# jaak-s/libfastsparse

Measured on AMD Instinct MI355X. Metric: fp64 CSR SpMV effective GB/s (% HBM3E peak), higher is better.
Workload: dtype f64

## Files before the change

libfastsparse_amd/csrc/fs_copies.hip:

```cpp
#include <algorithm>
#include <vector>

#include "fs_format_util.h"
#include "fs_plan.h"

namespace fs {

static_assert(sizeof(WorkItem) == sizeof(int4) && sizeof(RowLen) == sizeof(int2), "fs_plan.h's plain structs are the device's int4 / int2");

__global__ void piece_count_kernel(int nrow, int split, const int *__restrict__ row_ptr, int *__restrict__ cnt)
{
  const int r = blockIdx.x * blockDim.x + threadIdx.x;
  if (r > nrow) return;
  if (r == nrow) { cnt[r] = 0; return; }
  const int len = row_ptr[r + 1] - row_ptr[r];
  cnt[r] = len <= split ? 1 : (len + split - 1) / split;
}

__global__ void vrow_fill_kernel(int nrow, int split, const int *__restrict__ row_ptr, const int *__restrict__ vfirst,
                                 int *__restrict__ vrow_ptr)
{
  const int r = blockIdx.x * blockDim.x + threadIdx.x;
  if (r > nrow) return;
  if (r == nrow) { vrow_ptr[vfirst[nrow]] = row_ptr[nrow]; return; }
  const int a = row_ptr[r], v0 = vfirst[r], k = vfirst[r + 1] - v0;
  for (int i = 0; i < k; ++i) vrow_ptr[v0 + i] = a + i * split;
}

__device__ __forceinline__ int last_le(const int *__restrict__ a, int n, int64_t key)
{
  int lo = 0, hi = n;
  while (lo < hi) {
    const int mid = lo + ((hi - lo + 1) >> 1);
    if ((int64_t)a[mid] <= key) lo = mid; else hi = mid - 1;
  }
  return lo;
}

__global__ void tile_key_kernel(int nvrow, int64_t nnz, int P, int W, int J, const int *__restrict__ vrow_ptr,
                                const int *__restrict__ panel_row, const int *__restrict__ cols,
                                int *__restrict__ vrows, unsigned *__restrict__ keys)
{
  const int64_t i = (int64_t)blockIdx.x * blockDim.x + threadIdx.x;
  if (i >= nnz) return;
  const int v = last_le(vrow_ptr, nvrow, i);
  vrows[i] = v;
  const int p = last_le(panel_row, P, v);
  keys[i] = (unsigned)p * (unsigned)J + (unsigned)(cols[i] / W);
}

__global__ void tile_pack_kernel(int64_t nnz, int W, int J, int lcol_bits, const unsigned *__restrict__ skeys,
                                 const unsigned *__restrict__ perm, const int *__restrict__ vrows,
                                 const int *__restrict__ panel_row, const int *__restrict__ cols,
                                 const double *__restrict__ vals, unsigned *__restrict__ pk, double *__restrict__ vals_out)
{
  const int64_t i = (int64_t)blockIdx.x * blockDim.x + threadIdx.x;
  if (i >= nnz) return;
  const unsigned src = perm[i];
  const unsigned key = skeys[i];
  const unsigned p = key / (unsigned)J, j = key % (unsigned)J;
  const unsigned lrow = (unsigned)(vrows[src] - panel_row[p]), lcol = (unsigned)(cols[src] - (int)j * W);
  pk[i] = (lrow << lcol_bits) | lcol;
  if (vals) vals_out[i] = vals[src];
}

__global__ void max_row_len_kernel(int nrow, const int *__restrict__ row_ptr, int *__restrict__ out)
{
  const int r = blockIdx.x * blockDim.x + threadIdx.x;
  int len = r < nrow ? row_ptr[r + 1] - row_ptr[r] : 0;
  for (int m = 32; m > 0; m >>= 1) { const int o = __shfl_xor(len, m); len = o > len ? o : len; }
  if ((threadIdx.x & 63) == 0 && len > __hip_atomic_load(out, __ATOMIC_RELAXED, __HIP_MEMORY_SCOPE_AGENT)) atomicMax(out, len);
}

static int make_virtual_rows(const DeviceCsr &A, int split, hipStream_t s, Scratch<int> &vrow_ptr, int *nvrow_out,
                             int **vfirst_out, double **yv_out, int kw = 1)
{
  Scratch<int> cnt;
  Scratch<char> tmp;
  int nvrow = 0;
  FS_HIP(cnt.alloc((size_t)A.nrow + 1));
  FS_HIP(traced_malloc(vfirst_out, sizeof(int) * ((size_t)A.nrow + 1)));
  int *vfirst = *vfirst_out;
  hipLaunchKernelGGL(piece_count_kernel, dim3(grid_for((int64_t)A.nrow + 1)), dim3(256), 0, s, A.nrow, split, A.row_ptr,
                     cnt.p);
  FS_HIP(hipGetLastError());
  if (int rc = device_exclusive_scan(tmp, cnt.p, vfirst, (size_t)A.nrow + 1, s)) return rc;
  if (int rc = read_back(&nvrow, (const int *)vfirst + A.nrow, s)) return rc;
  FS_HIP(vrow_ptr.alloc((size_t)nvrow + 1));
  hipLaunchKernelGGL(vrow_fill_kernel, dim3(grid_for((int64_t)A.nrow + 1)), dim3(256), 0, s, A.nrow, split, A.row_ptr,
                     vfirst, vrow_ptr.p);
  FS_HIP(hipGetLastError());
  FS_HIP(traced_malloc(yv_out, sizeof(double) * (size_t)nvrow * (size_t)kw));
  *nvrow_out = nvrow;
  return FS_OK;
}

static int max_row_len(const DeviceCsr &A, hipStream_t s, int *out)
{
  if (A.max_row_len >= 0) { *out = A.max_row_len; return FS_OK; }
  Scratch<int> mx;
  FS_HIP(mx.alloc(1));
  FS_HIP(hipMemsetAsync(mx, 0, sizeof(int), s));
  hipLaunchKernelGGL(max_row_len_kernel, dim3(grid_for(A.nrow)), dim3(256), 0, s, A.nrow, A.row_ptr, mx.p);
  FS_HIP(hipGetLastError());
  if (int rc = read_back(out, (const int *)mx.p, s)) return rc;
  A.max_row_len = *out;
  return FS_OK;
}

struct VirtualRows {
  Scratch<int> own;
  const int *vrow_ptr = nullptr;
  int nvrow = 0;
  int split = 0;
  bool cut() const { return split > 0; }
  int fetch(std::vector<int> &vp, hipStream_t s) const
  {
    vp.resize((size_t)nvrow + 1);
    FS_HIP(hipMemcpyAsync(vp.data(), vrow_ptr, sizeof(int) * vp.size(), hipMemcpyDeviceToHost, s));
    FS_HIP(hipStreamSynchronize(s));
    return FS_OK;
  }
};

static int virtual_rows(const DeviceCsr &A, hipStream_t s, bool may_cut, int kw, VirtualRows &V, int **vfirst, double **yv)
{
  int max_len = 0;
  if (int rc = max_row_len(A, s, &max_len)) return rc;
  const int split = options().tile_split > 0 ? options().tile_split : 256;
  V.vrow_ptr = A.row_ptr;
  V.nvrow = A.nrow;
  if (may_cut && max_len > split) {
    V.split = split;
    if (int rc = make_virtual_rows(A, split, s, V.own, &V.nvrow, vfirst, yv, kw)) return rc;
    V.vrow_ptr = V.own.p;
  }
  return FS_OK;
}

static int sorted_runs(Scratch<char> &tmp, unsigned *keys, unsigned *skeys, unsigned *idx_in, unsigned *idx_out, size_t n, int64_t nruns,
                       int *run_ptr, hipStream_t s, const unsigned **sorted_keys, const unsigned **perm)
{
  if (int rc = device_iota((int64_t)n, idx_in, s)) return rc;
  if (int rc = device_sort_pairs(tmp, keys, skeys, idx_in, idx_out, n, sort_bits((uint64_t)nruns, 32), s, sorted_keys, perm)) return rc;
  return device_run_ptr(nruns, (int64_t)n, *sorted_keys, run_ptr, s);
}

__device__ __forceinline__ int rot_ffs(unsigned m, int rot)
{
  const unsigned rr = rot ? ((m >> rot) | (m << (32 - rot))) : m;
  return (__ffs((int)rr) - 1 + rot) & 31;
}

__device__ __forceinline__ void wave_lds_fence()
{
  __builtin_amdgcn_fence(__ATOMIC_SEQ_CST, "workgroup");
  __builtin_amdgcn_wave_barrier();
}

constexpr int kReorderThreads = 256;
constexpr int kReorderSegs = kReorderThreads / 32;
constexpr int kReorderPer = kTiledItem / kReorderThreads;

constexpr int kRepairMaxClass = 256;
constexpr int kRepairMaxGroup = 8;
constexpr int kRepairMaxLeft = 128;
constexpr int kRepairMaxBig = 96;

template <bool ARRANGE>
__global__ __launch_bounds__(kReorderThreads) void ldsx_reorder_kernel(const int4 *__restrict__ items, int lcol_bits,
                                                                      unsigned *__restrict__ pk, double *__restrict__ vals,
                                                                      int *__restrict__ bad, unsigned long long *__restrict__ clk)
{
  long long tick = clk ? clock64() : 0;
  auto lap = [&](int phase) {
    if (clk && threadIdx.x == 0) { const long long now = clock64(); atomicAdd(&clk[phase], (unsigned long long)(now - tick)); tick = now; }
  };
  __shared__ unsigned w[kTiledItem];
  __shared__ unsigned short lst[kTiledItem];
  __shared__ unsigned short seq[kTiledItem];
  __shared__ unsigned short segcnt[kReorderSegs][32 * 32];
  __shared__ unsigned short left[32 * 32];
  __shared__ unsigned short size[32 * 32];
  __shared__ unsigned short off[32 * 32];
  __shared__ int owner[32];
  static_assert(kReorderSegs * 32 * 32 >= 3 * kTiledItem + kTiledItem / 2, "the repair arrays are carved out of segcnt");
  unsigned short *const cplace = &segcnt[0][0];
  unsigned short *const crow = &segcnt[0][0] + kTiledItem;
  unsigned short *const lead = &segcnt[0][0] + 2 * kTiledItem;
  unsigned char *const flag = reinterpret_cast<unsigned char *>(&segcnt[0][0] + 3 * kTiledItem);
  __shared__ unsigned short unres[kRepairMaxLeft];
  __shared__ unsigned short pmem[kRepairMaxBig];
  __shared__ int nunres, ndup, wcount[32];
  const int4 d = items[blockIdx.x];
  const int n = d.y, t = threadIdx.x;
  for (int i = t; i < n; i += kReorderThreads) w[i] = pk[(int64_t)d.x + i];
  for (int i = t; i < kReorderSegs * 32 * 32; i += kReorderThreads) (&segcnt[0][0])[i] = 0;
  __syncthreads();
  {
    const int sg = t >> 5, c = t & 31;
    const int per = (n + kReorderSegs - 1) / kReorderSegs;
    const int i0 = sg * per, i1 = (i0 + per < n) ? i0 + per : n;
    for (int i = i0; i < i1; ++i)
      if ((int)((w[i] >> lcol_bits) & 31u) == c) {
        const int k = c * 32 + (ARRANGE ? (int)(w[i] & 31u) : 0);
        seq[i] = segcnt[sg][k]++;
      }
  }
  __syncthreads();
  lap(0);
  for (int k = t; k < 32 * 32; k += kReorderThreads) {
    int a = 0;
    for (int sg = 0; sg < kReorderSegs; ++sg) { const int m = segcnt[sg][k]; segcnt[sg][k] = (unsigned short)a; a += m; }
    size[k] = (unsigned short)a;
    left[k] = (unsigned short)a;
  }
  __syncthreads();
  unsigned avail = 0;
  int mine = 0;
  if (t < 64) {
    if (t < 32)
      for (int b = 0; b < 32; ++b) mine += size[t * 32 + b];
    int base = mine;
    for (int m = 1; m < 32; m <<= 1) {
      const int o = __shfl_up(base, m);
      if (t >= m) base += o;
    }
    base -= mine;
    if (t < 32) {
      int a = base;
      for (int b = 0; b < 32; ++b) {
        off[t * 32 + b] = (unsigned short)a;
        a += size[t * 32 + b];
        if (size[t * 32 + b]) avail |= 1u << b;
      }
    }
  }
  __syncthreads();
  {
    const int per = (n + kReorderSegs - 1) / kReorderSegs;
    for (int i = t; i < n; i += kReorderThreads) {
      const int k = (int)((w[i] >> lcol_bits) & 31u) * 32 + (ARRANGE ? (int)(w[i] & 31u) : 0);
      lst[off[k] + segcnt[i / per][k] + seq[i]] = (unsigned short)i;
    }
  }
  __syncthreads();
  lap(1);
  if (t < 64) {
    int remaining = t < 32 ? mine : 0, placed = 0;
    for (int r = 0;; ++r) {
      const unsigned nonempty = (unsigned)__ballot(remaining > 0);
      if (!nonempty) break;
      unsigned used = 0;
      int bank = -1;
      bool pending = remaining > 0;
      for (int iter = 0;; ++iter) {
        int prop = -1;
        if (pending) {
          const unsigned free_banks = avail & ~used;
          const int rot = (t + r + 7 * iter) & 31;
          if (!ARRANGE || free_banks == 0u) { bank = rot_ffs(avail, rot); pending = false; }
          else prop = rot_ffs(free_banks, rot);
        }
        if (!__ballot(prop >= 0)) break;
        if (t < 32) owner[t] = 255;
        wave_lds_fence();
        if (prop >= 0) atomicMin(&owner[prop], t);
        wave_lds_fence();
        if (prop >= 0 && owner[prop] == t) { bank = prop; pending = false; }
        used |= (unsigned)__ballot(t < 32 && owner[t & 31] != 255);
        wave_lds_fence();
      }
      if (bank >= 0) {
        const int k = t * 32 + bank;
        const int before = left[k];
        left[k] = (unsigned short)(before - 1);
        if (before == 1) avail &= ~(1u << bank);
        const int place = placed + __popc(nonempty & ((1u << t) - 1u));
        seq[place] = lst[off[k] + (size[k] - before)];
        cplace[off[t * 32] + (mine - remaining)] = (unsigned short)place;
        --remaining;
      }
      placed += __popc(nonempty);
    }
  }
  __syncthreads();
  lap(2);
  const int half = (n + 1) >> 1;
  {
    for (int g = t; g < n; g += kReorderThreads) crow[g] = (unsigned short)(w[seq[cplace[g]]] >> lcol_bits);
    __syncthreads();
    bool too_large = false;
    const int wv = __builtin_amdgcn_readfirstlane(t >> 6), lane = t & 63;
    auto rdlane = [](int v, int l) { return __builtin_amdgcn_readlane(v, __builtin_amdgcn_readfirstlane(l)); };
    for (int q8 = 0; q8 < 8; ++q8) {
      const int c = wv * 8 + q8;
      const int base = __builtin_amdgcn_readfirstlane((int)off[c * 32]);
      const int msize = __builtin_amdgcn_readfirstlane((c < 31 ? (int)off[(c + 1) * 32] : n) - base);
      const int m = msize < kRepairMaxClass ? msize : kRepairMaxClass;
      int row[4];
#pragma unroll
      for (int e = 0; e < 4; ++e) {
        const int idx = 64 * e + lane;
        row[e] = idx < m ? (int)crow[base + idx] : -1 - idx;
      }
#pragma unroll
      for (int e = 0; e < 4; ++e) {
        if (64 * e < m) {
          int first = -1;
#pragma unroll
          for (int e2 = 0; e2 < 4; ++e2) {
            if (e2 <= e) {
              const int lim = e2 < e ? 64 : lane;
              const int cnt = m - 64 * e2 < 64 ? m - 64 * e2 : 64;
              for (int l = 0; l < cnt; ++l) {
                const int rl = rdlane(row[e2], l);
                if (first < 0 && rl == row[e] && l < lim) first = 64 * e2 + l;
              }
            }
          }
          const int idx = 64 * e + lane;
          if (idx < m) {
            lead[base + idx] = (unsigned short)(base + (first < 0 ? idx : first));
            flag[base + idx] = 0;
          }
        }
      }
      for (int idx = kRepairMaxClass + lane; idx < msize; idx += 64) {
        lead[base + idx] = (unsigned short)(base + idx);
        flag[base + idx] = 0;
        too_large = true;
      }
    }
    __syncthreads();
    if (t == 0) { nunres = 0; ndup = 0; }
    __syncthreads();
    {
      int mydup = 0;
      for (int g = t; g < n; g += kReorderThreads)
        if (lead[g] != g) { flag[lead[g]] = 1; ++mydup; }
      if (mydup) atomicAdd(&ndup, mydup);
    }
    __syncthreads();
    lap(3);
    const bool hopeless = 4 * ndup > n && n > 128;
    bool failed = too_large || hopeless;
    auto wave_of = [&](int g) { const int sp = cplace[g]; return (sp < half ? sp : sp - half) >> 6; };
    auto trade = [&](int j, int k, int g) {
      const unsigned short ej = seq[cplace[j]], ek = seq[cplace[k]];
      seq[cplace[j]] = ek; seq[cplace[k]] = ej;
      const unsigned short rj = crow[j]; crow[j] = crow[k]; crow[k] = rj;
      lead[k] = (unsigned short)g; flag[k] = 2;
      lead[j] = (unsigned short)j; flag[j] = 0;
    };
    if (!hopeless) {
      for (int q8 = 0; q8 < 8; ++q8) {
        const int c = wv * 8 + q8;
        const int base = __builtin_amdgcn_readfirstlane((int)off[c * 32]);
        const int msize = __builtin_amdgcn_readfirstlane((c < 31 ? (int)off[(c + 1) * 32] : n) - base);
        const int m = msize < kRepairMaxClass ? msize : kRepairMaxClass;
        if (m <= 0) continue;
        int wof[4];
#pragma unroll
        for (int e = 0; e < 4; ++e) wof[e] = 64 * e + lane < m ? wave_of(base + 64 * e + lane) : 31;
        int myfree = 0;
        {
          bool fr[4];
#pragma unroll
          for (int e = 0; e < 4; ++e) {
            const int g = base + 64 * e + lane;
            fr[e] = 64 * e + lane < m && lead[g] == g && !(flag[g] & 3);
          }
          for (int v = 0; v < 16; ++v) {
            int cnt = 0;
#pragma unroll
            for (int e = 0; e < 4; ++e) cnt += __popcll(__ballot(fr[e] && wof[e] == v));
            if (lane == v) myfree = cnt;
          }
        }
        int cursor = -1;
        for (;;) {
          int G = -1;
#pragma unroll
          for (int e = 0; e < 4; ++e) {
            const int idx = 64 * e + lane, g = base + idx;
            const bool d = idx < m && idx > cursor && lead[g] == g && (flag[g] & 1) && !(flag[g] & 2);
            const unsigned long long mk = __ballot(d);
            if (G < 0 && mk) G = 64 * e + __ffsll((long long)mk) - 1;
          }
          if (G < 0) break;
          cursor = G;
          const int gG = base + G;
          bool mem[4];
          int gs = 0;
#pragma unroll
          for (int e = 0; e < 4; ++e) {
            mem[e] = 64 * e + lane < m && lead[base + 64 * e + lane] == gG;
            gs += __popcll(__ballot(mem[e]));
          }
          int best = -1;
          if (gs <= kRepairMaxGroup) {
            int have = 0;
#pragma unroll
            for (int e = 0; e < 4; ++e) {
              unsigned long long bits = __ballot(mem[e]);
              while (bits) {
                const int l = __ffsll((long long)bits) - 1;
                bits &= bits - 1;
                if (lane == rdlane(wof[e], l)) ++have;
              }
            }
            int key = (lane < 16 && have + myfree >= gs) ? ((have << 8) | (15 - lane)) : -1;
            for (int o = 32; o > 0; o >>= 1) { const int other = __shfl_xor(key, o); key = other > key ? other : key; }
            if (key >= 0) best = 15 - (key & 255);
          }
          if (best < 0) {
            if (lane == 0) {
              const int slot = atomicAdd(&nunres, 1);
              if (slot < kRepairMaxLeft) unres[slot] = (unsigned short)gG; else failed = true;
            }
            continue;
          }
#pragma unroll
          for (int e = 0; e < 4; ++e) {
            unsigned long long bits = __ballot(mem[e]);
            while (bits) {
              const int l = __ffsll((long long)bits) - 1;
              bits &= bits - 1;
              const int j = base + 64 * e + l;
              const int wj = rdlane(wof[e], l);
              if (wj == best) {
                if (lane == 0) flag[j] |= 2;
                wave_lds_fence();
                continue;
              }
              int k = -1;
#pragma unroll
              for (int e2 = 0; e2 < 4; ++e2) {
                const int g2 = base + 64 * e2 + lane;
                const bool f = 64 * e2 + lane < m && wof[e2] == best && lead[g2] == g2 && !(flag[g2] & 3);
                const unsigned long long fm = __ballot(f);
                if (k < 0 && fm) k = base + 64 * e2 + __ffsll((long long)fm) - 1;
              }
              if (k < 0) { failed = true; break; }
              if (lane == 0) trade(j, k, gG);
              wave_lds_fence();
              if (lane == best) --myfree;
              if (lane == wj) ++myfree;
            }
          }
          wave_lds_fence();
        }
      }
    }
    __syncthreads();
    {
      const int cnt = nunres < kRepairMaxLeft ? nunres : kRepairMaxLeft;
      int mine_u = 0, rank = 0;
      if (t < cnt) {
        mine_u = unres[t];
        for (int j = 0; j < cnt; ++j) rank += unres[j] < mine_u;
      }
      __syncthreads();
      if (t < cnt) unres[rank] = (unsigned short)mine_u;
    }
    __syncthreads();
    lap(4);
    {
      const int left = hopeless ? 0 : (nunres < kRepairMaxLeft ? nunres : kRepairMaxLeft);
      if (!hopeless && nunres > kRepairMaxLeft) failed = true;
      for (int u = 0; u < left; ++u) {
        const int g = unres[u];
        if (t < 32) wcount[t] = 0;
        __syncthreads();
        for (int j = t; j < n; j += kReorderThreads) {
          const int v = wave_of(j);
          if (lead[j] == g) atomicAdd(&wcount[v], 1);
          else if (lead[j] == j && !(flag[j] & 3)) atomicAdd(&wcount[16 + v], 1);
        }
        __syncthreads();
        if (t == 0 && !failed) {
          const int c = crow[g] & 31, base = off[c * 32];
          int m = (c < 31 ? (int)off[(c + 1) * 32] : n) - base;
          if (m > kRepairMaxClass) m = kRepairMaxClass;
          int gs = 0;
          for (int j = g; j < base + m; ++j)
            if (lead[j] == g) { if (gs < kRepairMaxBig) pmem[gs] = (unsigned short)j; ++gs; }
          int best = -1;
          for (int v = 0; v < 16; ++v)
            if (wcount[v] + wcount[16 + v] >= gs && (best < 0 || wcount[v] > wcount[best])) best = v;
          if (gs > kRepairMaxBig || best < 0) failed = true;
          else {
            int next = 0;
            for (int q = 0; q < gs; ++q) {
              const int j = pmem[q];
              if (wave_of(j) == best) { flag[j] |= 2; continue; }
              while (next < n && !(wave_of(next) == best && lead[next] == next && !(flag[next] & 3))) ++next;
              if (next >= n) { failed = true; break; }
              trade(j, next, g);
            }
          }
        }
        __syncthreads();
      }
    }
    if (failed) atomicAdd(bad, 1);
  }
  __syncthreads();
  lap(5);
  double v[kReorderPer];
#pragma unroll
  for (int j = 0; j < kReorderPer; ++j) {
    const int q = t + j * kReorderThreads;
    v[j] = (vals && q < n) ? vals[(int64_t)d.x + seq[q]] : 0.0;
  }
  __syncthreads();
#pragma unroll
  for (int j = 0; j < kReorderPer; ++j) {
    const int q = t + j * kReorderThreads;
    if (q < n) {
      const int pos = q < half ? 2 * q : 2 * (q - half) + 1;
      pk[(int64_t)d.x + pos] = w[seq[q]];
      if (vals) vals[(int64_t)d.x + pos] = v[j];
    }
  }
  lap(6);
}

constexpr int kPanelBandWords = 8192;
__global__ __launch_bounds__(256) void panel_bands_kernel(int stride, int W, int words, const int *__restrict__ panel_row,
                                                          const int *__restrict__ row_ptr, const int *__restrict__ cols,
                                                          int *__restrict__ out)
{
  __shared__ unsigned bits[kPanelBandWords];
  __shared__ int total;
  const int p = blockIdx.x * stride, t = threadIdx.x;
  for (int i = t; i < words; i += 256) bits[i] = 0u;
  if (t == 0) total = 0;
  __syncthreads();
  const int64_t e0 = row_ptr[panel_row[p]], e1 = row_ptr[panel_row[p + 1]];
  for (int64_t e = e0 + t; e < e1; e += 256) {
    const int b = cols[e] / W;
    atomicOr(&bits[b >> 5], 1u << (b & 31));
  }
  __syncthreads();
  int c = 0;
  for (int i = t; i < words; i += 256) c += __popc(bits[i]);
  atomicAdd(&total, c);
  __syncthreads();
  if (t == 0) { out[2 * blockIdx.x] = total; out[2 * blockIdx.x + 1] = (int)(e1 - e0); }
}

static int ldsx_sample_is_thin(const DeviceCsr &A, const int *vrow_ptr, const std::vector<int> &panel_row, int W, int J, hipStream_t s,
                               bool *thin)
{
  *thin = true;
  constexpr int kSample = 64;
  const int P = (int)panel_row.size() - 1, words = (J + 31) / 32;
  if (words > kPanelBandWords || P < 1) return FS_OK;
  const int ns = P < kSample ? P : kSample, stride = P / ns;
  Scratch<int> prow, cnt;
  FS_HIP(prow.alloc(panel_row.size()));
  FS_HIP(cnt.alloc(2 * (size_t)ns));
  FS_HIP(hipMemcpyAsync(prow.p, panel_row.data(), sizeof(int) * panel_row.size(), hipMemcpyHostToDevice, s));
  hipLaunchKernelGGL(panel_bands_kernel, dim3(ns), dim3(256), 0, s, stride, W, words, prow.p, vrow_ptr, A.cols, cnt.p);
  FS_HIP(hipGetLastError());
  std::vector<int> hc(2 * (size_t)ns);
  FS_HIP(hipMemcpyAsync(hc.data(), cnt.p, sizeof(int) * hc.size(), hipMemcpyDeviceToHost, s));
  FS_HIP(hipStreamSynchronize(s));
  *thin = ldsx_sample_thin(hc);
  return FS_OK;
}

static int reorder_ldsx_items(TiledCsr *T, hipStream_t s)
{
  static const bool arrange = [] { const char *v = getenv("FS_LDSX_ARRANGE"); return !(v && *v == '0'); }();
  static const bool profile = [] { const char *v = getenv("FS_LDSX_REORDER_PROFILE"); return v && *v == '1'; }();
  Scratch<int> bad;
  Scratch<unsigned long long> clk;
  FS_HIP(bad.alloc(1));
  FS_HIP(hipMemsetAsync(bad, 0, sizeof(int), s));
  if (profile) { FS_HIP(clk.alloc(8)); FS_HIP(hipMemsetAsync(clk, 0, 8 * sizeof(unsigned long long), s)); }
  if (arrange)
    hipLaunchKernelGGL(ldsx_reorder_kernel<true>, dim3(T->nitems), dim3(kReorderThreads), 0, s, T->items, T->lcol_bits, T->pk, T->vals, bad.p, profile ? clk.p : nullptr);
  else
    hipLaunchKernelGGL(ldsx_reorder_kernel<false>, dim3(T->nitems), dim3(kReorderThreads), 0, s, T->items, T->lcol_bits, T->pk, T->vals, bad.p, profile ? clk.p : nullptr);
  FS_HIP(hipGetLastError());
  if (profile) {
    unsigned long long h[8] = {};
    FS_HIP(hipMemcpyAsync(h, clk, sizeof h, hipMemcpyDeviceToHost, s));
    FS_HIP(hipStreamSynchronize(s));
    fprintf(stderr, "[fastsparse] ldsx_reorder_kernel, %d items, mean clocks per item: load+count %.0f, lists %.0f, rounds %.0f, repair rows+leaders %.0f, "
            "per class %.0f, leftovers %.0f, copy out %.0f\n", T->nitems, (double)h[0] / T->nitems, (double)h[1] / T->nitems, (double)h[2] / T->nitems,
            (double)h[3] / T->nitems, (double)h[4] / T->nitems, (double)h[5] / T->nitems, (double)h[6] / T->nitems);
  }
  int hbad = 0;
  if (int rc = read_back(&hbad, bad.p, s)) return rc;
  T->orderable = hbad == 0;
  if (trace_build() && hbad) fprintf(stderr, "[fastsparse] LDS-staged copy: %d of %d work items hold a row that does not fit one wave -- no fixed-order sums on this copy\n", hbad, T->nitems);
  return FS_OK;
}

static int upload_ldsx_chunks(TiledCsr *T, int nrow, const std::vector<int> &chunk_panel, const std::vector<int> &chunk_item,
                              const std::vector<int> &chunk_ord)
{
  const int P = T->P;
  T->nchunks = (int)chunk_panel.size();
  FS_HIP(traced_malloc(&T->chunk_panel, sizeof(int) * (chunk_panel.size() ? chunk_panel.size() : 1)));
  FS_HIP(traced_malloc(&T->chunk_item, sizeof(int) * (chunk_item.size() ? chunk_item.size() : 2)));
  FS_HIP(traced_malloc(&T->chunk_ord, sizeof(int) * (chunk_ord.size() ? chunk_ord.size() : 1)));
  {
    int *base = nullptr;
    FS_HIP(traced_malloc(&base, sizeof(int) * ((size_t)(P > 0 ? P : 1) + 1)));
    FS_HIP(hipMemset(base, 0, sizeof(int)));
    T->ticket = base + 1;
  }
  if (!chunk_panel.empty()) {
    FS_HIP(hipMemcpy(T->chunk_panel, chunk_panel.data(), sizeof(int) * chunk_panel.size(), hipMemcpyHostToDevice));
    FS_HIP(hipMemcpy(T->chunk_item, chunk_item.data(), sizeof(int) * chunk_item.size(), hipMemcpyHostToDevice));
    FS_HIP(hipMemcpy(T->chunk_ord, chunk_ord.data(), sizeof(int) * chunk_ord.size(), hipMemcpyHostToDevice));
  }
  if (T->shared && !T->yv) FS_HIP(traced_malloc(&T->yv, sizeof(double) * (size_t)nrow));
  return FS_OK;
}

static int build_tiled_impl(DeviceCsr &A, hipStream_t s, TiledCsr *&slot, bool ldsx)
{
  const Options &o = options();
  const int mode = ldsx ? o.ldsx : o.tiling;
  if (mode == 0 || A.nrow == 0 || A.nnz == 0) return FS_OK;
  const int ncu = cu_count();
  const int slots = (ncu > 8 ? ncu : 256) / 8 * 8;
  const int rows_max = ldsx ? kLdsxRows : kTiledRowsMax;

  const int64_t x_bytes = (int64_t)A.ncol * 8;
  if (mode == 1 && tiled_too_small(x_bytes, A.nnz)) return FS_OK;

  TiledCsr *T = new TiledCsr();
  slot = T;
  T->ldsx = ldsx;
  T->slots = slots; T->lcol_bits = kTiledColBits;
  VirtualRows V;
  if (int rc = virtual_rows(A, s, !ldsx, 1, V, &T->vfirst, &T->yv)) return rc;
  T->split = V.split;
  T->nvrow = V.nvrow;

  const int R = plan_tiled_rows(V.nvrow, slots, rows_max, ldsx, o.tile_rows);
  std::vector<int> vp;
  if (V.cut())
    if (int rc = V.fetch(vp, s)) return rc;
  const std::vector<int> panel_row = plan_tiled_panels(V.nvrow, R, V.cut(), vp, A.nnz, V.split);
  const int P = (int)panel_row.size() - 1;
  int W = 0, J = 0;
  plan_band_width(A.ncol, A.nnz, P, ldsx, o.tile_cols, &W, &J);
  const int64_t ntiles = (int64_t)P * J;
  if (mode == 1 && ldsx && ldsx_tiles_thin(A.nnz, ntiles)) {
    bool thin = true;
    if (int rc = ldsx_sample_is_thin(A, V.vrow_ptr, panel_row, W, J, s, &thin)) return rc;
    if (thin) return FS_OK;
  }
  if (mode == 1 && !ldsx && tiled_hopeless(A.nnz, ntiles, P, slots, x_bytes)) return FS_OK;
  if (ntiles >= (1ll << 31)) return FS_OK;
  T->R = R; T->W = W; T->P = P; T->J = J;
  T->entries_per_tile = (float)((double)A.nnz / (double)ntiles);
  FS_HIP(traced_malloc(&T->panel_row, sizeof(int) * panel_row.size()));
  FS_HIP(hipMemcpyAsync(T->panel_row, panel_row.data(), sizeof(int) * panel_row.size(), hipMemcpyHostToDevice, s));

  const size_t n = (size_t)A.nnz;
  Scratch<int> vrows, tile_ptr;
  Scratch<unsigned> keys, skeys, idx_in, idx_out;
  Scratch<char> tmp;
  FS_HIP(vrows.alloc(n));
  FS_HIP(keys.alloc(n));
  FS_HIP(skeys.alloc(n));
  FS_HIP(idx_in.alloc(n));
  FS_HIP(idx_out.alloc(n));
  FS_HIP(tile_ptr.alloc((size_t)ntiles + 1));
  FS_HIP(traced_malloc(&T->pk, sizeof(unsigned) * (n + 8)));
  if (A.vals) FS_HIP(traced_malloc(&T->vals, sizeof(double) * (n + 8)));
  hipLaunchKernelGGL(tile_key_kernel, dim3(grid_for(A.nnz)), dim3(256), 0, s, V.nvrow, A.nnz, P, W, J, V.vrow_ptr, T->panel_row,
                     A.cols, vrows.p, keys.p);
  const unsigned *sorted_keys = nullptr, *perm = nullptr;
  if (int rc = sorted_runs(tmp, keys.p, skeys.p, idx_in.p, idx_out.p, n, ntiles, tile_ptr.p, s, &sorted_keys, &perm)) return rc;
  hipLaunchKernelGGL(tile_pack_kernel, dim3(grid_for(A.nnz)), dim3(256), 0, s, A.nnz, W, J, T->lcol_bits, sorted_keys, perm,
                     vrows.p, T->panel_row, A.cols, A.vals, T->pk, T->vals);
  FS_HIP(hipGetLastError());
  std::vector<int> tp((size_t)ntiles + 1);
  FS_HIP(hipMemcpyAsync(tp.data(), tile_ptr.p, sizeof(int) * tp.size(), hipMemcpyDeviceToHost, s));
  FS_HIP(hipStreamSynchronize(s));
  std::vector<WorkItem> items;
  std::vector<int> item_ptr;
  cut_work_items(tp, P, J, items, item_ptr);
  T->nitems = (int)items.size();
  FS_HIP(traced_malloc(&T->items, sizeof(int4) * (items.size() ? items.size() : 1)));
  FS_HIP(traced_malloc(&T->item_ptr, sizeof(int) * item_ptr.size()));
  if (!items.empty()) FS_HIP(hipMemcpy(T->items, items.data(), sizeof(int4) * items.size(), hipMemcpyHostToDevice));
  FS_HIP(hipMemcpy(T->item_ptr, item_ptr.data(), sizeof(int) * item_ptr.size(), hipMemcpyHostToDevice));
  if (ldsx && T->nitems > 0)
    if (int rc = reorder_ldsx_items(T, s)) return rc;
  if (ldsx) {
    static const bool plain = [] { const char *v = getenv("FS_LDSX_ORDER"); return v && *v == '1'; }();
    std::vector<int> chunk_panel, chunk_item, chunk_ord;
    T->shared = plan_ldsx_chunks(item_ptr, (int64_t)items.size(), P, slots, plain, chunk_panel, chunk_item, chunk_ord);
    if (int rc = upload_ldsx_chunks(T, A.nrow, chunk_panel, chunk_item, chunk_ord)) return rc;
  }
  T->built = true;
  return FS_OK;
}

int build_tiled(DeviceCsr &A, hipStream_t s) { return optional_copy(build_tiled_impl(A, s, A.tiled, false), A.tiled, free_tiled_slot); }

int build_tiledx(DeviceCsr &A, hipStream_t s) { return optional_copy(build_tiled_impl(A, s, A.tiledx, true), A.tiledx, free_tiled_slot); }

__global__ void bin_key_kernel(int nvrow, int64_t nnz, int P, int bcols, const int *__restrict__ vrow_ptr,
                               const int *__restrict__ panel_row, const int *__restrict__ cols,
                               int *__restrict__ vrows, unsigned *__restrict__ keys)
{
  const int64_t i = (int64_t)blockIdx.x * blockDim.x + threadIdx.x;
  if (i >= nnz) return;
  const int v = last_le(vrow_ptr, nvrow, i);
  vrows[i] = v;
  keys[i] = (unsigned)(cols[i] / bcols) * (unsigned)P + (unsigned)last_le(panel_row, P, v);
}

__global__ void bin_groups_kernel(int B, int P, int ge, const int *__restrict__ run_ptr, unsigned *__restrict__ g1,
                                  unsigned *__restrict__ g2, const unsigned *__restrict__ xs = nullptr)
{
  const int64_t k = (int64_t)blockIdx.x * blockDim.x + threadIdx.x;
  const int64_t nruns = (int64_t)B * P;
  if (k > nruns) return;
  if (k == nruns) { g1[k] = 0; g2[k] = 0; return; }
  const int b = (int)(k / P), p = (int)(k % P);
  const unsigned dum = xs ? xs[run_ptr[k + 1]] - xs[run_ptr[k]] : 0u;
  const unsigned g = ((unsigned)(run_ptr[k + 1] - run_ptr[k]) + dum + (unsigned)ge - 1u) / (unsigned)ge;
  g1[k] = g;
  g2[(int64_t)p * B + b] = g;
}

__global__ void bin_scatter_kernel(int64_t nnz, int B, int P, int bcols, int ge, const unsigned *__restrict__ skeys,
                                   const unsigned *__restrict__ perm, const int *__restrict__ vrows,
                                   const int *__restrict__ panel_row, const int *__restrict__ cols,
                                   const double *__restrict__ vals, const int *__restrict__ run_ptr,
                                   const unsigned *__restrict__ start1, const unsigned *__restrict__ start2,
                                   uint16_t *__restrict__ lcol, double *__restrict__ vals1, uint16_t *__restrict__ lrow)
{
  const int64_t i = (int64_t)blockIdx.x * blockDim.x + threadIdx.x;
  if (i >= nnz) return;
  const unsigned key = skeys[i], src = perm[i];
  const int b = (int)(key / (unsigned)P), p = (int)(key % (unsigned)P);
  const int64_t rank = i - run_ptr[key];
  const int64_t pos1 = (int64_t)start1[key] * ge + rank;
  const int64_t pos2 = (int64_t)start2[(int64_t)p * B + b] * ge + rank;
  lcol[pos1] = (uint16_t)(cols[src] - b * bcols);
  if (vals) vals1[pos1] = vals[src];
  lrow[pos2] = (uint16_t)(vrows[src] - panel_row[p]);
}

__global__ void bin_gap_kernel(int64_t nnz, int P, const unsigned *__restrict__ skeys, const unsigned *__restrict__ perm,
                               const int *__restrict__ vrows, const int *__restrict__ run_ptr, unsigned *__restrict__ extra)
{
  const int64_t i = (int64_t)blockIdx.x * blockDim.x + threadIdx.x;
  if (i > nnz) return;
  if (i == nnz) { extra[i] = 0; return; }
  const unsigned key = skeys[i];
  unsigned e = 0;
  if (i > run_ptr[key]) {
    const int gap = vrows[perm[i]] - vrows[perm[i - 1]];
    if (gap > 255) e = (unsigned)(gap - 1) / 255u;
  }
  extra[i] = e;
}

__global__ void bin_scatter8_kernel(int64_t nnz, int B, int P, int bcols, int ge, const unsigned *__restrict__ skeys,
                                    const unsigned *__restrict__ perm, const int *__restrict__ vrows,
                                    const int *__restrict__ panel_row, const int *__restrict__ cols,
                                    const double *__restrict__ vals, const int *__restrict__ run_ptr,
                                    const unsigned *__restrict__ xs, const unsigned *__restrict__ start1,
                                    const unsigned *__restrict__ start2, uint16_t *__restrict__ lcol, double *__restrict__ vals1,
                                    uint8_t *__restrict__ lrow8, uint16_t *__restrict__ gbase)
{
  const int64_t i = (int64_t)blockIdx.x * blockDim.x + threadIdx.x;
  if (i >= nnz) return;
  const unsigned key = skeys[i], src = perm[i];
  const int b = (int)(key / (unsigned)P), p = (int)(key % (unsigned)P);
  const int64_t first = run_ptr[key];
  const unsigned dum = xs[i + 1] - xs[i];
  const int64_t slot = (i - first) + (int64_t)(xs[i] - xs[first]) + dum;
  const int64_t base1 = (int64_t)start1[key] * ge, base2 = (int64_t)start2[(int64_t)p * B + b] * ge;
  const int row = vrows[src] - panel_row[p];
  const int prev = i > first ? vrows[perm[i - 1]] - panel_row[p] : row;
  for (unsigned m = 0; m < dum; ++m) {
    const int64_t sl = slot - dum + m;
    lrow8[base2 + sl] = 255;
    if ((sl & (ge - 1)) == 0) gbase[(base2 + sl) / ge] = (uint16_t)(prev + 255 * (int)m);
  }
  const int before = prev + 255 * (int)dum;
  lcol[base1 + slot] = (uint16_t)(cols[src] - b * bcols);
  if (vals) vals1[base1 + slot] = vals[src];
  lrow8[base2 + slot] = (uint8_t)(row - before);
  if ((slot & (ge - 1)) == 0) gbase[(base2 + slot) / ge] = (uint16_t)before;
}

__global__ void bin_gdst_kernel(int B, int P, const unsigned *__restrict__ start1, const unsigned *__restrict__ start2,
                                unsigned *__restrict__ gdst)
{
  const int64_t k = (int64_t)blockIdx.x * blockDim.x + threadIdx.x;
  if (k >= (int64_t)B * P) return;
  const int b = (int)(k / P), p = (int)(k % P);
  const unsigned a = start1[k], n = start1[k + 1] - a, d = start2[(int64_t)p * B + b];
  for (unsigned j = 0; j < n; ++j) gdst[a + j] = d + j;
}

__global__ void bin_ptr_kernel(int B, int P, const unsigned *__restrict__ start1, const unsigned *__restrict__ start2,
                               unsigned *__restrict__ band_ptr, unsigned *__restrict__ bin_ptr)
{
  const int64_t k = (int64_t)blockIdx.x * blockDim.x + threadIdx.x;
  if (k <= B) band_ptr[k] = start1[k * P];
  if (k <= P) bin_ptr[k] = start2[k * B];
}

__global__ void long_candidates_kernel(int nrow, int minlen, const int *__restrict__ row_ptr, int *__restrict__ count, int cap,
                                       int2 *__restrict__ out)
{
  const int r = blockIdx.x * blockDim.x + threadIdx.x;
  if (r >= nrow) return;
  const int len = row_ptr[r + 1] - row_ptr[r];
  if (len < minlen) return;
  const int k = atomicAdd(count, 1);
  if (k < cap) out[k] = make_int2(r, len);
}

__global__ void long_mark_kernel(int nlong, const int *__restrict__ rows, int *__restrict__ row_to_long)
{
  const int i = blockIdx.x * blockDim.x + threadIdx.x;
  if (i < nlong) row_to_long[rows[i]] = i;
}

__global__ void main_len_kernel(int nrow, const int *__restrict__ row_ptr, const int *__restrict__ row_to_long, int *__restrict__ len)
{
  const int r = blockIdx.x * blockDim.x + threadIdx.x;
  if (r > nrow) return;
  len[r] = (r == nrow || row_to_long[r] >= 0) ? 0 : row_ptr[r + 1] - row_ptr[r];
}

__global__ void split_entries_kernel(int nrow, int64_t nnz, int nlong, int bcols, const int *__restrict__ row_ptr, const int *__restrict__ cols,
                                     const double *__restrict__ vals, const int *__restrict__ row_to_long,
                                     const int *__restrict__ main_rp, const int64_t *__restrict__ long_ptr,
                                     int *__restrict__ main_cols, double *__restrict__ main_vals, unsigned *__restrict__ lkey,
                                     unsigned *__restrict__ lsrc)
{
  const int64_t i = (int64_t)blockIdx.x * blockDim.x + threadIdx.x;
  if (i >= nnz) return;
  const int r = last_le(row_ptr, nrow, i);
  const int64_t k = i - row_ptr[r];
  const int l = row_to_long[r];
  if (l < 0) {
    const int64_t d = (int64_t)main_rp[r] + k;
    main_cols[d] = cols[i];
    if (vals) main_vals[d] = vals[i];
  } else {
    const int64_t d = long_ptr[l] + k;
    lkey[d] = (unsigned)(cols[i] / bcols) * (unsigned)nlong + (unsigned)l;
    lsrc[d] = (unsigned)i;
  }
}

__global__ void long_seg_start_kernel(int B, int nlong, int64_t n, const int *__restrict__ own_first, const unsigned *__restrict__ skeys,
                                      int64_t *__restrict__ start)
{
  const int64_t sg = (int64_t)blockIdx.x * blockDim.x + threadIdx.x;
  if (sg > (int64_t)B * kLongOwners) return;
  const int b = (int)(sg / kLongOwners), w = (int)(sg % kLongOwners);
  const uint64_t key = (uint64_t)b * (uint64_t)nlong + (uint64_t)(b < B ? own_first[w] : 0);
  int64_t lo = 0, hi = n;
  while (lo < hi) {
    const int64_t mid = lo + ((hi - lo) >> 1);
    if ((uint64_t)skeys[mid] < key) lo = mid + 1; else hi = mid;
  }
  start[sg] = lo;
}

__global__ void long_scatter_kernel(int64_t n, int nlong, int bcols, const unsigned *__restrict__ skeys, const unsigned *__restrict__ ssrc,
                                    const unsigned char *__restrict__ owner_of, const int64_t *__restrict__ shift,
                                    const int *__restrict__ cols, const double *__restrict__ vals, uint16_t *__restrict__ lcol,
                                    uint16_t *__restrict__ lrow, double *__restrict__ lvals)
{
  const int64_t k = (int64_t)blockIdx.x * blockDim.x + threadIdx.x;
  if (k >= n) return;
  const unsigned key = skeys[k], src = ssrc[k];
  const unsigned b = key / (unsigned)nlong, l = key - b * (unsigned)nlong;
  const int64_t d = k + shift[(int64_t)b * kLongOwners + owner_of[l]];
  lcol[d] = (uint16_t)(cols[src] - (int)b * bcols);
  lrow[d] = (uint16_t)l;
  if (lvals) lvals[d] = vals[src];
}

__global__ void long_pad_kernel(int64_t nseg, int bcols, const int64_t *__restrict__ start, const int64_t *__restrict__ shift,
                                uint16_t *__restrict__ lcol, uint16_t *__restrict__ lrow, double *__restrict__ lvals)
{
  const int64_t sg = (int64_t)blockIdx.x * blockDim.x + threadIdx.x;
  if (sg >= nseg) return;
  const int64_t cnt = start[sg + 1] - start[sg];
  if (cnt & 1) {
    const int64_t d = start[sg] + shift[sg] + cnt;
    lcol[d] = (uint16_t)bcols;
    lrow[d] = lrow[d - 1];
    if (lvals) lvals[d] = 0.0;
  }
}

static int split_long_rows(const DeviceCsr &A, hipStream_t s, LongRows **out, Scratch<int> &main_rp, Scratch<int> &main_cols,
                           Scratch<double> &main_vals, int64_t *main_nnz)
{
  *out = nullptr;
  const Options &o = options();
  if (o.long_rows == 0 || o.binning == 0 || A.nrow == 0 || A.nnz < (4 << 20)) return FS_OK;
  const bool narrow = o.long_geometry != 1;
  const int bcols = narrow ? kLongBandB : kLongBandA, cap_rows = narrow ? kLongRowsB : kLongRowsA;
  const int B = (A.ncol + bcols - 1) / bcols;
  const int minlen = o.long_min_len > 0 ? o.long_min_len : 512;
  constexpr int kCap = 1 << 18;
  Scratch<int> cnt;
  Scratch<int2> cand;
  FS_HIP(cnt.alloc(1));
  FS_HIP(cand.alloc(kCap));
  FS_HIP(hipMemsetAsync(cnt, 0, sizeof(int), s));
  hipLaunchKernelGGL(long_candidates_kernel, dim3(grid_for(A.nrow)), dim3(256), 0, s, A.nrow, minlen, A.row_ptr, cnt.p, kCap, cand.p);
  FS_HIP(hipGetLastError());
  int ncand = 0;
  if (int rc = read_back(&ncand, cnt.p, s)) return rc;
  if (ncand == 0 || ncand > kCap) return FS_OK;
  std::vector<RowLen> h((size_t)ncand);
  FS_HIP(hipMemcpy(h.data(), cand, sizeof(int2) * (size_t)ncand, hipMemcpyDeviceToHost));
  std::vector<int> rows, own_first;
  std::vector<unsigned char> owner_of;
  std::vector<int64_t> lptr;
  deal_long_rows(std::move(h), cap_rows, rows, own_first, owner_of, lptr);
  const int nlong = (int)rows.size();
  const int64_t nl = lptr[(size_t)nlong];
  if (o.long_rows == 1 && !long_rows_pay(nl, A.nnz, A.ncol)) return FS_OK;
  if ((uint64_t)B * (uint64_t)nlong >= (1ull << 32)) return FS_OK;

  LongRows *L = new LongRows();
  struct Guard { LongRows *&p; bool keep = false; ~Guard() { if (!keep) free_long_rows(p); } } guard{L};
  L->nlong = nlong; L->B = B; L->bcols = bcols;
  FS_HIP(traced_malloc(&L->row, sizeof(int) * (size_t)nlong));
  FS_HIP(hipMemcpyAsync(L->row, rows.data(), sizeof(int) * (size_t)nlong, hipMemcpyHostToDevice, s));
  FS_HIP(traced_malloc(&L->ylong, sizeof(double) * (size_t)nlong));

  Scratch<int> row_to_long, mlen;
  Scratch<int64_t> long_ptr, start, shift;
  Scratch<unsigned> lkey, lsrc, skey, ssrc;
  Scratch<char> tmp;
  FS_HIP(row_to_long.alloc((size_t)A.nrow));
  FS_HIP(mlen.alloc((size_t)A.nrow + 1));
  FS_HIP(main_rp.alloc((size_t)A.nrow + 1));
  FS_HIP(long_ptr.alloc((size_t)nlong + 1));
  FS_HIP(hipMemsetAsync(row_to_long, 0xff, sizeof(int) * (size_t)A.nrow, s));
  FS_HIP(hipMemcpyAsync(long_ptr, lptr.data(), sizeof(int64_t) * lptr.size(), hipMemcpyHostToDevice, s));
  hipLaunchKernelGGL(long_mark_kernel, dim3(grid_for(nlong)), dim3(256), 0, s, nlong, L->row, row_to_long.p);
  hipLaunchKernelGGL(main_len_kernel, dim3(grid_for((int64_t)A.nrow + 1)), dim3(256), 0, s, A.nrow, A.row_ptr, row_to_long.p, mlen.p);
  FS_HIP(hipGetLastError());
  if (int rc = device_exclusive_scan(tmp, mlen.p, main_rp.p, (size_t)A.nrow + 1, s)) return rc;
  const int64_t nm = A.nnz - nl;
  *main_nnz = nm;
  FS_HIP(main_cols.alloc((size_t)(nm > 0 ? nm : 1)));
  if (A.vals) FS_HIP(main_vals.alloc((size_t)(nm > 0 ? nm : 1)));
  FS_HIP(lkey.alloc((size_t)nl));
  FS_HIP(lsrc.alloc((size_t)nl));
  FS_HIP(skey.alloc((size_t)nl));
  FS_HIP(ssrc.alloc((size_t)nl));
  hipLaunchKernelGGL(split_entries_kernel, dim3(grid_for(A.nnz)), dim3(256), 0, s, A.nrow, A.nnz, nlong, bcols, A.row_ptr, A.cols, A.vals,
                     row_to_long.p, main_rp.p, long_ptr.p, main_cols.p, A.vals ? main_vals.p : nullptr, lkey.p, lsrc.p);
  FS_HIP(hipGetLastError());
  Scratch<char> tmp2;
  const unsigned *sorted_keys = nullptr, *sorted_src = nullptr;
  if (int rc = device_sort_pairs(tmp2, lkey.p, skey.p, lsrc.p, ssrc.p, (size_t)nl, sort_bits((uint64_t)B * (uint64_t)nlong, 32), s,
                                 &sorted_keys, &sorted_src)) return rc;
  const int64_t nseg = (int64_t)B * kLongOwners;
  Scratch<int> d_own_first;
  Scratch<unsigned char> d_owner_of;
  FS_HIP(start.alloc((size_t)nseg + 1));
  FS_HIP(shift.alloc((size_t)nseg + 1));
  FS_HIP(d_own_first.alloc((size_t)kLongOwners + 1));
  FS_HIP(d_owner_of.alloc((size_t)nlong));
  FS_HIP(hipMemcpyAsync(d_own_first, own_first.data(), sizeof(int) * own_first.size(), hipMemcpyHostToDevice, s));
  FS_HIP(hipMemcpyAsync(d_owner_of, owner_of.data(), owner_of.size(), hipMemcpyHostToDevice, s));
  hipLaunchKernelGGL(long_seg_start_kernel, dim3(grid_for(nseg + 1)), dim3(256), 0, s, B, nlong, nl, d_own_first.p, sorted_keys, start.p);
  FS_HIP(hipGetLastError());
  std::vector<int64_t> hs((size_t)nseg + 1), hp, hsh;
  std::vector<unsigned> hseg;
  FS_HIP(hipMemcpyAsync(hs.data(), start, sizeof(int64_t) * hs.size(), hipMemcpyDeviceToHost, s));
  FS_HIP(hipStreamSynchronize(s));
  if (!pad_long_segments(hs, B, hp, hseg, hsh)) return FS_OK;
  L->n = hp[(size_t)B];
  FS_HIP(traced_malloc(&L->band_ptr, sizeof(int64_t) * ((size_t)B + 1)));
  FS_HIP(traced_malloc(&L->seg_ptr, sizeof(unsigned) * hseg.size()));
  FS_HIP(hipMemcpyAsync(L->band_ptr, hp.data(), sizeof(int64_t) * hp.size(), hipMemcpyHostToDevice, s));
  FS_HIP(hipMemcpyAsync(L->seg_ptr, hseg.data(), sizeof(unsigned) * hseg.size(), hipMemcpyHostToDevice, s));
  FS_HIP(hipMemcpyAsync(shift, hsh.data(), sizeof(int64_t) * hsh.size(), hipMemcpyHostToDevice, s));
  FS_HIP(traced_malloc(&L->lcol, sizeof(uint16_t) * (size_t)(L->n + 2)));
  FS_HIP(traced_malloc(&L->lrow, sizeof(uint16_t) * (size_t)(L->n + 2)));
  if (A.vals) FS_HIP(traced_malloc(&L->vals, sizeof(double) * (size_t)(L->n + 2)));
  hipLaunchKernelGGL(long_scatter_kernel, dim3(grid_for(nl)), dim3(256), 0, s, nl, nlong, bcols, sorted_keys, sorted_src, d_owner_of.p,
                     shift.p, A.cols, A.vals, L->lcol, L->lrow, L->vals);
  hipLaunchKernelGGL(long_pad_kernel, dim3(grid_for(nseg)), dim3(256), 0, s, nseg, bcols, start.p, shift.p, L->lcol, L->lrow, L->vals);
  FS_HIP(hipGetLastError());
  const int ncu = cu_count();
  const int64_t by_size = (L->n + kBinShareMin - 1) / kBinShareMin;
  L->nwg = (int)(by_size < ncu ? by_size : ncu);
  FS_HIP(traced_malloc(&L->ypart, sizeof(double) * (size_t)(L->nwg > 0 ? L->nwg : 1) * (size_t)nlong));
  FS_HIP(hipStreamSynchronize(s));
  guard.keep = true;
  *out = L;
  return FS_OK;
}

static int build_binned_impl(DeviceCsr &A, hipStream_t s, BinnedCsr *&slot, int kw)
{
  const Options &o = options();
  static const int big_env = [] { const char *v = getenv("FS_BIN_BIG"); return v && *v ? atoi(v) : -1; }();
  const TwoPassGeometry g = plan_two_pass_geometry(A.nrow, A.ncol, A.nnz, kw, o.bin_rows, big_env);
  const int bcols = g.bcols, ge = g.ge;
  if (o.binning == 0 || A.nrow == 0 || A.nnz == 0) return FS_OK;
  if (o.binning == 1 && A.nnz < (4 << 20)) return FS_OK;
  const int ncu = cu_count();
  const int slots = ncu > 0 ? ncu : 256;

  BinnedCsr *N = new BinnedCsr();
  slot = N;
  N->kw = kw;
  N->bcols = bcols;
  VirtualRows V;
  if (int rc = virtual_rows(A, s, true, kw, V, &N->vfirst, &N->yv)) return rc;
  N->split = V.split;
  N->nvrow = V.nvrow;
  const int nvrow = V.nvrow;

  std::vector<int> vp;
  if (int rc = V.fetch(vp, s)) return rc;
  static const double fill = [] { const char *v = getenv("FS_BIN_FILL"); return v && *v ? atof(v) / 100.0 : 0.8; }();
  static const int min_panels = [] { const char *v = getenv("FS_BIN_MIN_PANELS"); return v && *v ? atoi(v) : 1; }();
  const std::vector<int> panel_row = plan_two_pass_panels(vp, nvrow, A.nnz, g.R, slots, fill, min_panels, kw);
  const int P = (int)panel_row.size() - 1;
  const int B = (A.ncol + bcols - 1) / bcols;
  const int64_t nruns = (int64_t)P * B;
  if (nruns >= (1ll << 28)) return FS_OK;
  if (o.binning == 1 && two_pass_padding_dominates(A.nnz, nruns, ge)) return FS_OK;
  N->P = P; N->B = B; N->slots = slots;
  FS_HIP(traced_malloc(&N->panel_row, sizeof(int) * panel_row.size()));
  FS_HIP(hipMemcpyAsync(N->panel_row, panel_row.data(), sizeof(int) * panel_row.size(), hipMemcpyHostToDevice, s));

  const size_t n = (size_t)A.nnz;
  Scratch<int> vrows, run_ptr;
  Scratch<unsigned> keys, skeys, idx_in, idx_out, g1, g2, start1, start2;
  Scratch<char> tmp, tmp2;
  FS_HIP(vrows.alloc(n));
  FS_HIP(keys.alloc(n));
  FS_HIP(skeys.alloc(n));
  FS_HIP(idx_in.alloc(n));
  FS_HIP(idx_out.alloc(n));
  FS_HIP(run_ptr.alloc((size_t)nruns + 1));
  FS_HIP(g1.alloc((size_t)nruns + 1));
  FS_HIP(g2.alloc((size_t)nruns + 1));
  FS_HIP(start1.alloc((size_t)nruns + 1));
  FS_HIP(start2.alloc((size_t)nruns + 1));
  FS_HIP(traced_malloc(&N->band_ptr, sizeof(unsigned) * ((size_t)B + 1)));
  FS_HIP(traced_malloc(&N->bin_ptr, sizeof(unsigned) * ((size_t)P + 1)));
  hipLaunchKernelGGL(bin_key_kernel, dim3(grid_for(A.nnz)), dim3(256), 0, s, nvrow, A.nnz, P, bcols, V.vrow_ptr, N->panel_row,
                     A.cols, vrows.p, keys.p);
  const unsigned *sorted_keys = nullptr, *perm = nullptr;
  if (int rc = sorted_runs(tmp, keys.p, skeys.p, idx_in.p, idx_out.p, n, nruns, run_ptr.p, s, &sorted_keys, &perm)) return rc;
  Scratch<unsigned> extra, xs;
  Scratch<char> tmp3;
  bool rows8 = false;
  int64_t dummies = 0;
  if (kw == 1 && bcols == kBinCols && !(o.bin_flags & 64) && A.nnz > 0) {
    FS_HIP(extra.alloc(n + 1));
    FS_HIP(xs.alloc(n + 1));
    hipLaunchKernelGGL(bin_gap_kernel, dim3(grid_for(A.nnz + 1)), dim3(256), 0, s, A.nnz, P, sorted_keys, perm, vrows.p, run_ptr.p, extra.p);
    FS_HIP(hipGetLastError());
    if (int rc = device_exclusive_scan(tmp3, extra.p, xs.p, n + 1, s)) return rc;
    unsigned total = 0;
    if (int rc = read_back(&total, (const unsigned *)xs.p + n, s)) return rc;
    dummies = total;
    rows8 = (o.bin_flags & 128) || (double)total <= 0.01 * (double)A.nnz;
  }
  hipLaunchKernelGGL(bin_groups_kernel, dim3(grid_for(nruns + 1)), dim3(256), 0, s, B, P, ge, run_ptr.p, g1.p, g2.p,
                     rows8 ? (const unsigned *)xs.p : (const unsigned *)nullptr);
  FS_HIP(hipGetLastError());
  if (int rc = device_exclusive_scan(tmp2, g1.p, start1.p, (size_t)nruns + 1, s)) return rc;
  if (int rc = device_exclusive_scan(tmp2, g2.p, start2.p, (size_t)nruns + 1, s)) return rc;
  hipLaunchKernelGGL(bin_ptr_kernel, dim3(grid_for((B > P ? B : P) + 1)), dim3(256), 0, s, B, P, start1.p, start2.p, N->band_ptr,
                     N->bin_ptr);
  FS_HIP(hipGetLastError());
  unsigned total_groups = 0;
  if (int rc = read_back(&total_groups, (const unsigned *)N->band_ptr + B, s)) return rc;
  const int64_t groups = total_groups;
  if (groups >= (1ll << 28) * (int64_t)kw) return FS_OK;
  if (groups >= (1ll << 32) - 1) return FS_OK;
  N->n = groups * ge;
  if (o.binning == 1 && kw == 1 && two_pass_hopeless(N->n, A.vals != nullptr, B, ncu, bcols, nvrow, A.ncol, A.nnz)) return FS_OK;

  const size_t np = (size_t)N->n;
  FS_HIP(traced_malloc(&N->lcol, sizeof(uint16_t) * np));
  if (rows8) {
    FS_HIP(traced_malloc(&N->lrow8, np));
    FS_HIP(traced_malloc(&N->gbase, sizeof(uint16_t) * (size_t)(groups ? groups : 1)));
    N->dummies = dummies;
  } else {
    FS_HIP(traced_malloc(&N->lrow, sizeof(uint16_t) * np));
  }
  FS_HIP(traced_malloc(&N->gdst, sizeof(unsigned) * (size_t)groups));
  FS_HIP(traced_malloc(&N->prod, sizeof(double) * np * (size_t)kw));
  if (A.vals) {
    FS_HIP(traced_malloc(&N->vals, sizeof(double) * np));
    FS_HIP(hipMemsetAsync(N->vals, 0, sizeof(double) * np, s));
  }
  FS_HIP(hipMemsetD16Async((hipDeviceptr_t)N->lcol, (unsigned short)bcols, np, s));
  if (rows8) {
    FS_HIP(hipMemsetAsync(N->lrow8, 0, np, s));
    FS_HIP(hipMemsetAsync(N->gbase, 0, sizeof(uint16_t) * (size_t)(groups ? groups : 1), s));
    hipLaunchKernelGGL(bin_scatter8_kernel, dim3(grid_for(A.nnz)), dim3(256), 0, s, A.nnz, B, P, bcols, ge, sorted_keys, perm, vrows.p,
                       N->panel_row, A.cols, A.vals, run_ptr.p, xs.p, start1.p, start2.p, N->lcol, N->vals, N->lrow8, N->gbase);
  } else {
    FS_HIP(hipMemsetAsync(N->lrow, 0, sizeof(uint16_t) * np, s));
    hipLaunchKernelGGL(bin_scatter_kernel, dim3(grid_for(A.nnz)), dim3(256), 0, s, A.nnz, B, P, bcols, ge, sorted_keys, perm, vrows.p,
                       N->panel_row, A.cols, A.vals, run_ptr.p, start1.p, start2.p, N->lcol, N->vals, N->lrow);
  }
  hipLaunchKernelGGL(bin_gdst_kernel, dim3(grid_for(nruns)), dim3(256), 0, s, B, P, start1.p, start2.p, N->gdst);
  FS_HIP(hipGetLastError());

  {
    const int64_t by_size = (N->n * kw + kBinShareMin - 1) / kBinShareMin;
    N->nwg1 = (int)(by_size < ncu ? by_size : ncu);
  }
  FS_HIP(hipStreamSynchronize(s));
  N->built = true;
  return FS_OK;
}

int build_binned(DeviceCsr &A, hipStream_t s)
{
  LongRows *lr = nullptr;
  Scratch<int> main_rp, main_cols;
  Scratch<double> main_vals;
  int64_t main_nnz = 0;
  if (split_long_rows(A, s, &lr, main_rp, main_cols, main_vals, &main_nnz) != FS_OK) {
    free_long_rows(lr);
    (void)hipGetLastError();
  }
  int rc;
  if (lr) {
    DeviceCsr M;
    M.nrow = A.nrow; M.ncol = A.ncol; M.nnz = main_nnz;
    M.row_ptr = main_rp.p; M.cols = main_cols.p; M.vals = A.vals ? main_vals.p : nullptr; M.owns = false;
    rc = build_binned_impl(M, s, A.binned, 1);
    if (rc == FS_OK && A.binned && A.binned->built) { A.binned->lr = lr; lr = nullptr; }
    M = DeviceCsr();
  } else {
    rc = build_binned_impl(A, s, A.binned, 1);
  }
  free_long_rows(lr);
  return optional_copy(rc, A.binned, free_binned_slot);
}

int build_binned_k(DeviceCsr &A, int kw, hipStream_t s)
{
  if (kw != 2 && kw != 4) return FS_ERR_ARG;
  BinnedCsr *&slot = kw == 2 ? A.binned2 : A.binned4;
  (kw == 2 ? A.tried2 : A.tried4) = true;
  return optional_copy(build_binned_impl(A, s, slot, kw), slot, free_binned_slot);
}

constexpr double kTiledBestEntriesPerMs = 152e6;

template <typename F>
static int time_product(F launch, hipStream_t s, hipEvent_t e0, hipEvent_t e1, float *median, int reps = 5)
{
  float t[5] = {1e30f, 1e30f, 1e30f, 1e30f, 1e30f};
  for (int rep = -1; rep < reps; ++rep) {
    FS_HIP(hipEventRecord(e0, s));
    if (int rc = launch()) return rc;
    FS_HIP(hipEventRecord(e1, s));
    FS_HIP(hipEventSynchronize(e1));
    float ms = 0.f;
    FS_HIP(hipEventElapsedTime(&ms, e0, e1));
    if (rep >= 0) t[rep] = ms;
  }
  std::sort(t, t + reps);
  *median = t[reps / 2];
  return FS_OK;
}

int two_pass_clear_win(DeviceCsr &A, hipStream_t s, bool *win)
{
  *win = false;
  const Options &o = options();
  if (!(A.binned && A.binned->built) || o.binning != 1 || o.tiling != 1 || A.nnz < (32ll << 20) || 8.0 * (double)A.ncol <= (double)(4 << 20)) return FS_OK;
  Scratch<double> x, y;
  if (x.alloc((size_t)A.ncol) != hipSuccess || y.alloc((size_t)A.nrow) != hipSuccess) { (void)hipGetLastError(); return FS_OK; }
  FS_HIP(hipMemsetAsync(x, 0, sizeof(double) * (size_t)A.ncol, s));
  hipEvent_t e0, e1;
  FS_HIP(hipEventCreate(&e0));
  if (hipEventCreate(&e1) != hipSuccess) { (void)hipEventDestroy(e0); return FS_OK; }
  float t = 1e30f;
  const int rc = time_product([&] { return launch_spmv_binned(A, y, x, s); }, s, e0, e1, &t, 2);
  (void)hipEventDestroy(e0);
  (void)hipEventDestroy(e1);
  if (rc != FS_OK) return rc;
  *win = (double)t <= (double)A.nnz / (A.vals ? kTiledBestEntriesPerMs : 200e6);
  return FS_OK;
}

int choose_copy(DeviceCsr &A, hipStream_t s)
{
  BuildClock clock(s);
  const Options &o = options();
  const bool hb = A.binned && A.binned->built, ht = A.tiled && A.tiled->built, hx = A.tiledx && A.tiledx->built;
  if (!hb && !ht && !hx) return FS_OK;
  if (o.tiling == 2 || o.binning == 2 || o.ldsx == 2) {
    if (o.binning != 2) free_binned_slot(A.binned);
    if (o.ldsx != 2) free_tiled_slot(A.tiledx);
    if (o.tiling != 2) free_tiled_slot(A.tiled);
    return FS_OK;
  }
  Scratch<double> x, y;
  if (x.alloc((size_t)A.ncol) != hipSuccess || y.alloc((size_t)A.nrow) != hipSuccess) {
    (void)hipGetLastError();
    return FS_OK;
  }
  FS_HIP(hipMemsetAsync(x, 0, sizeof(double) * (size_t)A.ncol, s));
  hipEvent_t e0, e1;
  FS_HIP(hipEventCreate(&e0));
  if (hipEventCreate(&e1) != hipSuccess) { (void)hipEventDestroy(e0); return FS_OK; }
  float t_stream = 1e30f, t_tiled = 1e30f, t_bin = 1e30f, t_ldsx = 1e30f;
  const bool lone_ldsx = hx && !hb && !ht && A.tiledx->entries_per_tile >= kLdsxClearWin;
  int rc = time_product([&] { return launch_spmv(A, y, x, s, true); }, s, e0, e1, &t_stream, (lone_ldsx || A.two_pass_clear_win) ? 1 : 5);
  if (rc == FS_OK && ht) rc = time_product([&] { return launch_spmv_tiled(A, *A.tiled, y, x, s); }, s, e0, e1, &t_tiled);
  if (rc == FS_OK && hx) rc = time_product([&] { return launch_spmv_tiled(A, *A.tiledx, y, x, s); }, s, e0, e1, &t_ldsx);
  if (rc == FS_OK && hb) rc = time_product([&] { return launch_spmv_binned(A, y, x, s); }, s, e0, e1, &t_bin);
  (void)hipEventDestroy(e0);
  (void)hipEventDestroy(e1);
  if (rc != FS_OK) return rc;
  A.build_ms[6] = clock.lap();
  A.candidate_ms[0] = t_stream;
  A.candidate_ms[1] = ht ? t_tiled : 0.f;
  A.candidate_ms[2] = hx ? t_ldsx : 0.f;
  A.candidate_ms[3] = hb ? t_bin : 0.f;
  float best = t_stream;
  if (t_tiled < best) best = t_tiled;
  if (t_ldsx < best) best = t_ldsx;
  if (t_bin < best) best = t_bin;
  const float tie = best * 1.05f;
  const int keep = (hb && t_bin <= tie) ? 3 : (hx && t_ldsx <= tie) ? 2 : (ht && t_tiled <= tie) ? 1 : 0;
  if (keep != 3) free_binned_slot(A.binned);
  if (keep != 2) free_tiled_slot(A.tiledx);
  if (keep != 1) free_tiled_slot(A.tiled);
  A.build_ms[7] = clock.lap();
  return FS_OK;
}

}
```

libfastsparse_amd/csrc/fs_kernels_twopass.hip:

```cpp
#include <stdlib.h>

#include "fs_kernel_util.h"

namespace fs {


template <bool VALUED, int U, bool NTLD, bool NTST, int BC>
__device__ __forceinline__ void expand_share(double *__restrict__ xband, int ncol, int B, const unsigned *__restrict__ band_ptr,
                                             const uint16_t *__restrict__ lcol, const double *__restrict__ vals,
                                             const unsigned *__restrict__ gdst, const double *__restrict__ x, int xs,
                                             double *__restrict__ prod, unsigned g0, unsigned g1)
{
  const int t = threadIdx.x;
  if (g0 >= g1) return;
  int b;
  {
    int lo = 0, hi = B - 1;
    while (lo < hi) {
      const int mid = lo + ((hi - lo + 1) >> 1);
      if (band_ptr[mid] <= g0) lo = mid; else hi = mid - 1;
    }
    b = lo;
  }
  for (unsigned g = g0; g < g1; ++b) {
    const unsigned gb = band_ptr[b + 1] < g1 ? band_ptr[b + 1] : g1;
    if (gb <= g) continue;
    const int c0 = b * BC;
    const int w = (ncol - c0 < BC) ? ncol - c0 : BC;
    __syncthreads();
    {
      double r[BC / kBinBlock];
#pragma unroll
      for (int j = 0; j < BC / kBinBlock; ++j) {
        const int i = j * kBinBlock + t;
        r[j] = __builtin_nontemporal_load(x + (int64_t)(c0 + (i < w ? i : w - 1)) * xs);
      }
#pragma unroll
      for (int j = 0; j < BC / kBinBlock; ++j) {
        const int i = j * kBinBlock + t;
        xband[i] = (i < w) ? r[j] : 0.0;
      }
      if (t < 8) xband[BC + t] = 0.0;
    }
    __syncthreads();
    const int64_t e0 = (int64_t)g * kBinGroup, e1 = (int64_t)gb * kBinGroup;
    constexpr int64_t kRound = 2 * U * kBinBlock;
    int64_t o = e0 + 2 * t;
    for (; o - 2 * t + kRound <= e1; o += kRound) {
      unsigned a[U], d[U];
      v2d v[U];
#pragma unroll
      for (int k = 0; k < U; ++k) {
        const int64_t e = o + (int64_t)k * 2 * kBinBlock;
        a[k] = stream_load<NTLD>((const unsigned *)(lcol + e));
        d[k] = stream_load<NTLD>(gdst + (e >> kBinGroupLog));
        if (VALUED) v[k] = stream_load<NTLD>((const v2d *)(vals + e));
      }
      __builtin_amdgcn_sched_barrier(0);
#pragma unroll
      for (int k = 0; k < U; ++k) {
        const int64_t e = o + (int64_t)k * 2 * kBinBlock;
        v2d p = {xband[a[k] & 0xffffu], xband[a[k] >> 16]};
        if (VALUED) { p.x *= v[k].x; p.y *= v[k].y; }
        stream_store<NTST>(p, (v2d *)(prod + (int64_t)d[k] * kBinGroup + (e & (kBinGroup - 1))));
      }
    }
    for (; o < e1; o += 2 * kBinBlock) {
      const unsigned a = stream_load<NTLD>((const unsigned *)(lcol + o));
      const unsigned d = stream_load<NTLD>(gdst + (o >> kBinGroupLog));
      v2d p = {xband[a & 0xffffu], xband[a >> 16]};
      if (VALUED) {
        const v2d v = stream_load<NTLD>((const v2d *)(vals + o));
        p.x *= v.x; p.y *= v.y;
      }
      stream_store<NTST>(p, (v2d *)(prod + (int64_t)d * kBinGroup + (o & (kBinGroup - 1))));
    }
    g = gb;
  }
}

template <bool VALUED, int U, bool NTLD, bool NTST, int BC = kBinCols>
__global__ __launch_bounds__(kBinBlock) void spmv_expand_kernel(
    int ncol, int B, const unsigned *__restrict__ band_ptr, const uint16_t *__restrict__ lcol,
    const double *__restrict__ vals, const unsigned *__restrict__ gdst, const double *__restrict__ x, int xs,
    double *__restrict__ prod, unsigned gbeg, unsigned gend)
{
  __shared__ double xband[BC + 8];
  const uint64_t groups = gend - gbeg;
  const unsigned g0 = gbeg + (unsigned)(groups * blockIdx.x / gridDim.x), g1 = gbeg + (unsigned)(groups * (blockIdx.x + 1) / gridDim.x);
  expand_share<VALUED, U, NTLD, NTST, BC>(xband, ncol, B, band_ptr, lcol, vals, gdst, x, xs, prod, g0, g1);
}

template <bool NTLD, bool L8>
__device__ __forceinline__ v4u row_ids_load(const uint16_t *__restrict__ lrow, const uint8_t *__restrict__ lrow8,
                                            const uint16_t *__restrict__ gbase, int64_t e)
{
  if (!L8) return stream_load<NTLD>((const v4u *)(lrow + e));
  typedef unsigned v2u __attribute__((ext_vector_type(2)));
  const v2u d = stream_load<NTLD>((const v2u *)(lrow8 + e));
  return v4u{d.x, d.y, (unsigned)gbase[e >> kBinGroupLog], (unsigned)(e >> 3) & 1u};
}

template <bool L8>
__device__ __forceinline__ v4u row_ids(v4u raw)
{
  if (!L8) return raw;
  const unsigned dx = raw.x, dy = raw.y;
  const unsigned s0 = dx & 0xffu, s1 = s0 + ((dx >> 8) & 0xffu), s2 = s1 + ((dx >> 16) & 0xffu), s3 = s2 + (dx >> 24);
  const unsigned s4 = s3 + (dy & 0xffu), s5 = s4 + ((dy >> 8) & 0xffu), s6 = s5 + ((dy >> 16) & 0xffu), s7 = s6 + (dy >> 24);
  const unsigned below = (unsigned)__builtin_amdgcn_update_dpp(0, (int)s7, 0x111 , 0xf, 0xf, false);
  const unsigned off = raw.z + (raw.w ? below : 0u);
  return v4u{(off + s0) | ((off + s1) << 16), (off + s2) | ((off + s3) << 16), (off + s4) | ((off + s5) << 16), (off + s6) | ((off + s7) << 16)};
}

template <bool L8>
__device__ __forceinline__ unsigned line_ids_load(const uint16_t *__restrict__ lrow, const uint8_t *__restrict__ lrow8,
                                                  const uint16_t *__restrict__ gbase, int64_t e)
{
  if (!L8) return *(const unsigned *)(lrow + e);
  return (unsigned)*(const uint16_t *)(lrow8 + e) | ((unsigned)gbase[e >> kBinGroupLog] << 16);
}

template <bool L8>
__device__ __forceinline__ unsigned line_ids(unsigned raw)
{
  if (!L8) return raw;
  const unsigned d0 = raw & 0xffu, own = d0 + ((raw >> 8) & 0xffu), l = threadIdx.x & 7u;
  unsigned s = own, u;
  u = (unsigned)__builtin_amdgcn_update_dpp(0, (int)s, 0x111 , 0xf, 0xf, false); s += l >= 1 ? u : 0u;
  u = (unsigned)__builtin_amdgcn_update_dpp(0, (int)s, 0x112 , 0xf, 0xf, false); s += l >= 2 ? u : 0u;
  u = (unsigned)__builtin_amdgcn_update_dpp(0, (int)s, 0x114 , 0xf, 0xf, false); s += l >= 4 ? u : 0u;
  const unsigned off = (raw >> 16) + s - own;
  return (off + d0) | ((off + own) << 16);
}

template <bool NTLD, bool L8 = false>
__device__ __forceinline__ void reduce_panel(double *__restrict__ ytile, int panel, const unsigned *__restrict__ bin_ptr,
                                             const int *__restrict__ panel_row, const uint16_t *__restrict__ lrow,
                                             const double *__restrict__ prod, double *__restrict__ y, int ys,
                                             const uint8_t *__restrict__ lrow8 = nullptr, const uint16_t *__restrict__ gbase = nullptr)
{
  const int t = threadIdx.x;
  const int r0 = panel_row[panel], nr = panel_row[panel + 1] - r0;
  for (int i = t; i < nr; i += kBinBlock) ytile[i] = 0.0;
  __syncthreads();
  const int64_t e0 = (int64_t)bin_ptr[panel] * kBinGroup, e1 = (int64_t)bin_ptr[panel + 1] * kBinGroup;
#define FS_ADD(idx, val) __hip_atomic_fetch_add(&ytile[idx], val, __ATOMIC_RELAXED, __HIP_MEMORY_SCOPE_WORKGROUP)
#define FS_ADD2(A, P) FS_ADD((A) & 0xffffu, (P).x); FS_ADD((A) >> 16, (P).y);
  constexpr int64_t kStep = 8 * kBinBlock, kRound = 2 * kStep;
  const int wave0 = (t >> 6) * 512, lane0 = wave0 + 2 * (t & 63);
  int64_t eb = e0;
  for (; eb + kRound <= e1; eb += kRound) {
    const int64_t e = eb + lane0;
    unsigned a[2][4];
    v2d p[2][4];
#pragma unroll
    for (int k = 0; k < 2; ++k)
#pragma unroll
      for (int j = 0; j < 4; ++j) {
        const int64_t ek = e + k * kStep + 128 * j;
        a[k][j] = line_ids_load<L8>(lrow, lrow8, gbase, ek);
        p[k][j] = stream_load<NTLD>((const v2d *)(prod + ek));
      }
    __builtin_amdgcn_sched_barrier(0);
#pragma unroll
    for (int k = 0; k < 2; ++k)
#pragma unroll
      for (int j = 0; j < 4; ++j) {
        const unsigned r = line_ids<L8>(a[k][j]);
        FS_ADD2(r, p[k][j])
      }
  }
  for (; eb + wave0 < e1; eb += kStep) {
    const int64_t e = eb + lane0;
    unsigned a[4];
    v2d p[4];
#pragma unroll
    for (int j = 0; j < 4; ++j) {
      const int64_t ej = e + 128 * j, ec = ej < e1 ? ej : e1 - 2;
      a[j] = line_ids_load<L8>(lrow, lrow8, gbase, ec);
      p[j] = stream_load<NTLD>((const v2d *)(prod + ec));
    }
#pragma unroll
    for (int j = 0; j < 4; ++j) {
      const unsigned r = line_ids<L8>(a[j]);
      if (e + 128 * j < e1) { FS_ADD2(r, p[j]) }
    }
  }
#undef FS_ADD2
#undef FS_ADD
  __syncthreads();
  for (int i = t; i < nr; i += kBinBlock) y[(int64_t)(r0 + i) * ys] = ytile[i];
}

template <bool NTLD, int RM = kBinRowsMax, bool L8 = false>
__global__ __launch_bounds__(kBinBlock) void spmv_reduce_kernel(
    const unsigned *__restrict__ bin_ptr, const int *__restrict__ panel_row, const uint16_t *__restrict__ lrow,
    const double *__restrict__ prod, double *__restrict__ y, int ys, int pbase, const uint8_t *__restrict__ lrow8 = nullptr,
    const uint16_t *__restrict__ gbase = nullptr)
{
  __shared__ double ytile[RM];
  reduce_panel<NTLD, L8>(ytile, pbase + blockIdx.x, bin_ptr, panel_row, lrow, prod, y, ys, lrow8, gbase);
}

#ifndef FS_ORDERED_DEPTH
#define FS_ORDERED_DEPTH 16
#endif
template <bool NTLD, int RM, int DEPTH, bool L8 = false>
__global__ __launch_bounds__(64) void spmv_reduce_ordered_kernel(
    const unsigned *__restrict__ bin_ptr, const int *__restrict__ panel_row, const uint16_t *__restrict__ lrow,
    const double *__restrict__ prod, double *__restrict__ y, int ys, int pbase, const uint8_t *__restrict__ lrow8 = nullptr,
    const uint16_t *__restrict__ gbase = nullptr)
{
  __shared__ __attribute__((aligned(16))) double ytile[RM];
  const int t = threadIdx.x;
  const int panel = pbase + blockIdx.x;
  const int r0 = panel_row[panel], nr = panel_row[panel + 1] - r0;
  for (int i = 2 * t; i < nr; i += 128) *reinterpret_cast<v2d *>(&ytile[i]) = v2d{0.0, 0.0};
  const int64_t e0 = (int64_t)bin_ptr[panel] * kBinGroup, e1 = (int64_t)bin_ptr[panel + 1] * kBinGroup;
#define FS_ADD(idx, val) __hip_atomic_fetch_add(&ytile[idx], val, __ATOMIC_RELAXED, __HIP_MEMORY_SCOPE_WORKGROUP)
#define FS_ADD8(A, P)                                                  \
  FS_ADD(A.x & 0xffffu, P[0].x); FS_ADD(A.x >> 16, P[0].y);            \
  FS_ADD(A.y & 0xffffu, P[1].x); FS_ADD(A.y >> 16, P[1].y);            \
  FS_ADD(A.z & 0xffffu, P[2].x); FS_ADD(A.z >> 16, P[2].y);            \
  FS_ADD(A.w & 0xffffu, P[3].x); FS_ADD(A.w >> 16, P[3].y);
  constexpr int64_t kStep = 8 * 64;
  v4u a[DEPTH];
  v2d p[DEPTH][4];
  auto fetch = [&](int k, int64_t e) {
    const int64_t ec = (e + 8 <= e1) ? e : (e1 - e0 >= 8 ? e1 - 8 : e0);
    a[k] = row_ids_load<NTLD, L8>(lrow, lrow8, gbase, ec);
#pragma unroll
    for (int j = 0; j < 4; ++j) p[k][j] = stream_load<NTLD>((const v2d *)(prod + ec + 2 * j));
  };
  if (e1 > e0) {
    int64_t e = e0 + 8 * t;
#pragma unroll
    for (int k = 0; k < DEPTH; ++k) fetch(k, e + (int64_t)k * kStep);
    for (; e - 8 * t < e1; e += (int64_t)DEPTH * kStep) {
#pragma unroll
      for (int k = 0; k < DEPTH; ++k) {
        const int64_t ek = e + (int64_t)k * kStep;
        const v4u ak = row_ids<L8>(a[k]);
        v2d pk[4] = {p[k][0], p[k][1], p[k][2], p[k][3]};
        fetch(k, ek + (int64_t)DEPTH * kStep);
        if (ek + 8 <= e1) { FS_ADD8(ak, pk) }
      }
    }
  }
#undef FS_ADD8
#undef FS_ADD
  __syncthreads();
  for (int i = t; i < nr; i += 64) y[(int64_t)(r0 + i) * ys] = ytile[i];
}

template <bool VALUED, int BC, int NACC, bool ORDERED>
__global__ __launch_bounds__(kBinBlock) void spmv_longrows_kernel(
    int ncol, int B, int nlong, const int64_t *__restrict__ band_ptr, const unsigned *__restrict__ seg_ptr,
    const uint16_t *__restrict__ lcol, const uint16_t *__restrict__ lrow, const double *__restrict__ vals,
    const double *__restrict__ x, int xs, double *__restrict__ ylong, double *__restrict__ ypart)
{
  __shared__ double xband[BC + 8];
  __shared__ double acc[NACC];
  const int t = threadIdx.x, lane = t & 63, wave = t >> 6;
  for (int i = t; i < nlong; i += kBinBlock) acc[i] = 0.0;
  const int64_t pairs = band_ptr[B] >> 1;
  const int64_t e_beg = 2 * (pairs * blockIdx.x / gridDim.x), e_end = 2 * (pairs * (blockIdx.x + 1) / gridDim.x);
  if (e_beg < e_end) {
    int b;
    {
      int lo = 0, hi = B - 1;
      while (lo < hi) {
        const int mid = lo + ((hi - lo + 1) >> 1);
        if (band_ptr[mid] <= e_beg) lo = mid; else hi = mid - 1;
      }
      b = lo;
    }
    double rn[BC / kBinBlock];
    int have = -1;
    auto request = [&](int bb) {
      const int cb = bb * BC;
      const int wb = (ncol - cb < BC) ? ncol - cb : BC;
#pragma unroll
      for (int j = 0; j < BC / kBinBlock; ++j) {
        const int i = j * kBinBlock + t;
        rn[j] = __builtin_nontemporal_load(x + (int64_t)(cb + (i < wb ? i : wb - 1)) * xs);
      }
      have = bb;
    };
    auto wave_step = [&](int64_t o, bool live, int64_t oc) {
      const unsigned a = *reinterpret_cast<const unsigned *>(lcol + oc);
      const unsigned rr = *reinterpret_cast<const unsigned *>(lrow + oc);
      v2d p = {xband[a & 0xffffu], xband[a >> 16]};
      if (VALUED) { const v2d v = *reinterpret_cast<const v2d *>(vals + oc); p.x *= v.x; p.y *= v.y; }
      unsigned key = 0xffffffffu;
      double sum = 0.0;
      if (live) {
        const unsigned r0 = rr & 0xffffu, r1 = rr >> 16;
        if (r0 == r1) { key = r0; sum = p.x + p.y; }
        else { __hip_atomic_fetch_add(&acc[r0], p.x, __ATOMIC_RELAXED, __HIP_MEMORY_SCOPE_WORKGROUP); key = r1; sum = p.y; }
      }
#pragma unroll
      for (int d = 1; d < 64; d <<= 1) {
        const unsigned ku = __shfl_up(key, d);
        const double su = __shfl_up(sum, d);
        if (lane >= d && ku == key) sum += su;
      }
      const unsigned kn = __shfl_down(key, 1);
      if (live && (lane == 63 || kn != key))
        __hip_atomic_fetch_add(&acc[key], sum, __ATOMIC_RELAXED, __HIP_MEMORY_SCOPE_WORKGROUP);
      (void)o;
    };
    for (int64_t e = e_beg; e < e_end; ++b) {
      const int64_t eb = band_ptr[b + 1] < e_end ? band_ptr[b + 1] : e_end;
      if (eb <= e) continue;
      const int c0 = b * BC;
      const int w = (ncol - c0 < BC) ? ncol - c0 : BC;
      if (have != b) request(b);
      __syncthreads();
#pragma unroll
      for (int j = 0; j < BC / kBinBlock; ++j) {
        const int i = j * kBinBlock + t;
        xband[i] = (i < w) ? rn[j] : 0.0;
      }
      if (t < 8) xband[BC + t] = 0.0;
      __syncthreads();
      if (b + 1 < B && eb < e_end) request(b + 1);
      if (ORDERED) {
        const int64_t s0 = band_ptr[b] + seg_ptr[b * (kLongOwners + 1) + wave], s1 = band_ptr[b] + seg_ptr[b * (kLongOwners + 1) + wave + 1];
        const int64_t lo = s0 > e ? s0 : e, hi = s1 < eb ? s1 : eb;
        for (int64_t o0 = lo; o0 < hi; o0 += 128) {
          const int64_t o = o0 + 2 * lane;
          const bool live = o < hi;
          wave_step(o, live, live ? o : lo);
        }
      } else {
        for (int64_t o0 = e; o0 < eb; o0 += 2 * kBinBlock) {
          const int64_t o = o0 + 2 * t;
          const bool live = o < eb;
          wave_step(o, live, live ? o : e);
        }
      }
      e = eb;
    }
  }
  __syncthreads();
  if (ORDERED) {
    double *__restrict__ mine = ypart + (int64_t)blockIdx.x * nlong;
    for (int i = t; i < nlong; i += kBinBlock) mine[i] = acc[i];
  } else {
    for (int i = t; i < nlong; i += kBinBlock) {
      const double v = acc[i];
      if (v != 0.0) unsafeAtomicAdd(ylong + i, v);
    }
  }
}

__global__ __launch_bounds__(kBlock) void longrows_combine_kernel(int nlong, int nwg, const double *__restrict__ ypart, double *__restrict__ ylong)
{
  const int i = blockIdx.x * kBlock + threadIdx.x;
  if (i >= nlong) return;
  double acc = 0.0;
  for (int w = 0; w < nwg; ++w) acc += ypart[(int64_t)w * nlong + i];
  ylong[i] = acc;
}

__global__ __launch_bounds__(kBlock) void longrows_scatter_kernel(int nlong, const int *__restrict__ row, const double *__restrict__ ylong,
                                                                 double *__restrict__ y, int ys, int row0, int row1)
{
  const int i = blockIdx.x * kBlock + threadIdx.x;
  if (i >= nlong) return;
  const int r = row[i];
  if (r >= row0 && r < row1) y[(int64_t)r * ys] = 0.0 + ylong[i];
}

static int launch_longrows(const DeviceCsr &A, const LongRows &L, const double *x, int xs, hipStream_t s)
{
  const bool ordered = reproducible_now();
  if (!ordered || L.n == 0 || L.nwg == 0)
    if (int rc = launch_zero(L.ylong, sizeof(double) * (size_t)L.nlong, s)) return rc;
  if (L.n == 0 || L.nwg == 0) return FS_OK;
#define FS_LONG(V, BC, NA, ORD)                                                                                              \
  hipLaunchKernelGGL((spmv_longrows_kernel<V, BC, NA, ORD>), dim3(L.nwg), dim3(kBinBlock), 0, s, A.ncol, L.B, L.nlong, L.band_ptr, \
                     L.seg_ptr, L.lcol, L.lrow, L.vals, x, xs, L.ylong, L.ypart)
#define FS_LONG2(V, BC, NA) do { if (ordered) FS_LONG(V, BC, NA, true); else FS_LONG(V, BC, NA, false); } while (0)
  if (L.bcols == kLongBandB) { if (A.has_vals()) FS_LONG2(true, kLongBandB, kLongRowsB); else FS_LONG2(false, kLongBandB, kLongRowsB); }
  else                       { if (A.has_vals()) FS_LONG2(true, kLongBandA, kLongRowsA); else FS_LONG2(false, kLongBandA, kLongRowsA); }
#undef FS_LONG2
#undef FS_LONG
  FS_HIP(hipGetLastError());
  if (ordered) {
    hipLaunchKernelGGL(longrows_combine_kernel, dim3((unsigned)((L.nlong + kBlock - 1) / kBlock)), dim3(kBlock), 0, s, L.nlong, L.nwg, L.ypart,
                       L.ylong);
    FS_HIP(hipGetLastError());
  }
  return FS_OK;
}


template <bool VALUED, int K, int U>
__global__ __launch_bounds__(kBinBlock) void spmm_expand_kernel(
    int ncol, int B, const unsigned *__restrict__ band_ptr, const uint16_t *__restrict__ lcol,
    const double *__restrict__ vals, const unsigned *__restrict__ gdst, const double *__restrict__ X, int xs,
    double *__restrict__ prod)
{
  constexpr int BC = kBinCols / K;
  constexpr int GE = kBinGroup / K;
  constexpr int LP = K / 2;
  constexpr int EPS = kBinBlock / LP;
  __shared__ __attribute__((aligned(16))) double xband[kBinCols + 8];
  const int t = threadIdx.x;
  const int le = t / LP, h = t % LP;
  const uint64_t groups = band_ptr[B];
  const unsigned g0 = (unsigned)(groups * blockIdx.x / gridDim.x), g1 = (unsigned)(groups * (blockIdx.x + 1) / gridDim.x);
  if (g0 >= g1) return;
  int b;
  {
    int lo = 0, hi = B - 1;
    while (lo < hi) {
      const int mid = lo + ((hi - lo + 1) >> 1);
      if (band_ptr[mid] <= g0) lo = mid; else hi = mid - 1;
    }
    b = lo;
  }
  for (unsigned g = g0; g < g1; ++b) {
    const unsigned gb = band_ptr[b + 1] < g1 ? band_ptr[b + 1] : g1;
    if (gb <= g) continue;
    const int c0 = b * BC;
    const int w = (ncol - c0 < BC) ? ncol - c0 : BC;
    __syncthreads();
    {
      double r[kBinCols / kBinBlock];
#pragma unroll
      for (int j = 0; j < kBinCols / kBinBlock; ++j) {
        const int f = j * kBinBlock + t, i = f / K, q = f % K;
        r[j] = __builtin_nontemporal_load(X + (int64_t)(c0 + (i < w ? i : w - 1)) * xs + q);
      }
#pragma unroll
      for (int j = 0; j < kBinCols / kBinBlock; ++j) {
        const int f = j * kBinBlock + t;
        xband[f] = (f / K < w) ? r[j] : 0.0;
      }
      if (t < 8) xband[kBinCols + t] = 0.0;
    }
    __syncthreads();
    const int64_t e0 = (int64_t)g * GE, e1 = (int64_t)gb * GE;
    constexpr int64_t kRound = (int64_t)U * EPS;
    int64_t o = e0 + le;
    for (; o - le + kRound <= e1; o += kRound) {
      unsigned a[U], d[U];
      double v[U];
#pragma unroll
      for (int k = 0; k < U; ++k) {
        const int64_t e = o + (int64_t)k * EPS;
        a[k] = lcol[e];
        d[k] = gdst[e / GE];
        if (VALUED) v[k] = vals[e];
      }
      __builtin_amdgcn_sched_barrier(0);
#pragma unroll
      for (int k = 0; k < U; ++k) {
        const int64_t e = o + (int64_t)k * EPS;
        v2d p = *reinterpret_cast<const v2d *>(&xband[a[k] * K + 2 * h]);
        if (VALUED) { p.x *= v[k]; p.y *= v[k]; }
        __builtin_nontemporal_store(p, (v2d *)(prod + ((int64_t)d[k] * GE + (e % GE)) * K + 2 * h));
      }
    }
    for (; o < e1; o += EPS) {
      const unsigned a = lcol[o];
      const unsigned d = gdst[o / GE];
      v2d p = *reinterpret_cast<const v2d *>(&xband[a * K + 2 * h]);
      if (VALUED) { const double v = vals[o]; p.x *= v; p.y *= v; }
      __builtin_nontemporal_store(p, (v2d *)(prod + ((int64_t)d * GE + (o % GE)) * K + 2 * h));
    }
    g = gb;
  }
}

template <int K>
__global__ __launch_bounds__(kBinBlock) void spmm_reduce_kernel(
    const unsigned *__restrict__ bin_ptr_all, const int *__restrict__ panel_row_all, const uint16_t *__restrict__ lrow,
    const double *__restrict__ prod, double *__restrict__ Y, int ys, int pbase)
{
  const unsigned *__restrict__ bin_ptr = bin_ptr_all + pbase;
  const int *__restrict__ panel_row = panel_row_all + pbase;
  constexpr int GE = kBinGroup / K;
  constexpr int EPL = 8 / K;
  __shared__ double ytile[kBinRowsMax];
  const int t = threadIdx.x;
  const int r0 = panel_row[blockIdx.x], nr = panel_row[blockIdx.x + 1] - r0;
  for (int i = t; i < nr * K; i += kBinBlock) ytile[i] = 0.0;
  __syncthreads();
  const int64_t e0 = (int64_t)bin_ptr[blockIdx.x] * GE, e1 = (int64_t)bin_ptr[blockIdx.x + 1] * GE;
  typedef uint16_t rows_t __attribute__((ext_vector_type(EPL)));
#define FS_ADD(idx, val) __hip_atomic_fetch_add(&ytile[idx], val, __ATOMIC_RELAXED, __HIP_MEMORY_SCOPE_WORKGROUP)
  auto add8 = [&](const rows_t a, const v2d (&p)[4]) {
#pragma unroll
    for (int q = 0; q < EPL; ++q) {
      const int base = (int)a[q] * K;
#pragma unroll
      for (int j = 0; j < K; j += 2) {
        FS_ADD(base + j, p[(q * K + j) / 2].x);
        FS_ADD(base + j + 1, p[(q * K + j) / 2].y);
      }
    }
  };
  constexpr int64_t kStep = (int64_t)EPL * kBinBlock;
  constexpr int64_t kRound = 2 * kStep;
  int64_t e = e0 + (int64_t)EPL * t;
  for (; e - EPL * t + kRound <= e1; e += kRound) {
    rows_t a[2];
    v2d p[2][4];
#pragma unroll
    for (int k = 0; k < 2; ++k) {
      const int64_t ek = e + k * kStep;
      a[k] = *reinterpret_cast<const rows_t *>(lrow + ek);
#pragma unroll
      for (int j = 0; j < 4; ++j) p[k][j] = *reinterpret_cast<const v2d *>(prod + ek * K + 2 * j);
    }
    __builtin_amdgcn_sched_barrier(0);
    add8(a[0], p[0]);
    add8(a[1], p[1]);
  }
  for (; e < e1; e += kStep) {
    const rows_t a = *reinterpret_cast<const rows_t *>(lrow + e);
    v2d p[4];
#pragma unroll
    for (int j = 0; j < 4; ++j) p[j] = *reinterpret_cast<const v2d *>(prod + e * K + 2 * j);
    add8(a, p);
  }
#undef FS_ADD
  __syncthreads();
  for (int i = t; i < nr * K; i += kBinBlock) Y[(int64_t)(r0 + i / K) * ys + (i % K)] = ytile[i];
}

template <int K, int DEPTH>
__global__ __launch_bounds__(64) void spmm_reduce_ordered_kernel(
    const unsigned *__restrict__ bin_ptr_all, const int *__restrict__ panel_row_all, const uint16_t *__restrict__ lrow,
    const double *__restrict__ prod, double *__restrict__ Y, int ys, int pbase)
{
  const unsigned *__restrict__ bin_ptr = bin_ptr_all + pbase;
  const int *__restrict__ panel_row = panel_row_all + pbase;
  constexpr int GE = kBinGroup / K;
  constexpr int EPL = 8 / K;
  __shared__ double ytile[kBinRowsMax];
  const int t = threadIdx.x;
  const int r0 = panel_row[blockIdx.x], nr = panel_row[blockIdx.x + 1] - r0;
  for (int i = t; i < nr * K; i += 64) ytile[i] = 0.0;
  const int64_t e0 = (int64_t)bin_ptr[blockIdx.x] * GE, e1 = (int64_t)bin_ptr[blockIdx.x + 1] * GE;
  typedef uint16_t rows_t __attribute__((ext_vector_type(EPL)));
#define FS_ADD(idx, val) __hip_atomic_fetch_add(&ytile[idx], val, __ATOMIC_RELAXED, __HIP_MEMORY_SCOPE_WORKGROUP)
  auto add8 = [&](const rows_t a, const v2d (&p)[4]) {
#pragma unroll
    for (int q = 0; q < EPL; ++q) {
      const int base = (int)a[q] * K;
#pragma unroll
      for (int j = 0; j < K; j += 2) {
        FS_ADD(base + j, p[(q * K + j) / 2].x);
        FS_ADD(base + j + 1, p[(q * K + j) / 2].y);
      }
    }
  };
  constexpr int64_t kStep = (int64_t)EPL * 64;
  rows_t a[DEPTH];
  v2d p[DEPTH][4];
  auto fetch = [&](int k, int64_t e) {
    const int64_t ec = (e + EPL <= e1) ? e : (e1 - e0 >= EPL ? e1 - EPL : e0);
    a[k] = *reinterpret_cast<const rows_t *>(lrow + ec);
#pragma unroll
    for (int j = 0; j < 4; ++j) p[k][j] = *reinterpret_cast<const v2d *>(prod + ec * K + 2 * j);
  };
  if (e1 > e0) {
    int64_t e = e0 + (int64_t)EPL * t;
#pragma unroll
    for (int k = 0; k < DEPTH; ++k) fetch(k, e + (int64_t)k * kStep);
    for (; e - EPL * t < e1; e += (int64_t)DEPTH * kStep) {
#pragma unroll
      for (int k = 0; k < DEPTH; ++k) {
        const int64_t ek = e + (int64_t)k * kStep;
        const rows_t ak = a[k];
        const v2d pk[4] = {p[k][0], p[k][1], p[k][2], p[k][3]};
        fetch(k, ek + (int64_t)DEPTH * kStep);
        if (ek + EPL <= e1) add8(ak, pk);
      }
    }
  }
#undef FS_ADD
  __syncthreads();
  for (int i = t; i < nr * K; i += 64) Y[(int64_t)(r0 + i / K) * ys + (i % K)] = ytile[i];
}

template <int K>
__global__ __launch_bounds__(kBlock) void tiled_combine_k_kernel(int nrow, const int *__restrict__ vfirst,
                                                                const double *__restrict__ yv, double *__restrict__ Y, int ys,
                                                                int row0 = 0)
{
  const int64_t i = (int64_t)row0 * K + (int64_t)blockIdx.x * kBlock + threadIdx.x;
  const int64_t r = i / K;
  const int j = (int)(i % K);
  if (r >= nrow) return;
  const int a = vfirst[r], b = vfirst[r + 1];
  double acc = yv[(int64_t)a * K + j];
  for (int v = a + 1; v < b; ++v) acc += yv[(int64_t)v * K + j];
  Y[r * ys + j] = acc;
}

__global__ void rows8_decode_kernel(int64_t groups, const uint8_t *__restrict__ lrow8, const uint16_t *__restrict__ gbase,
                                    uint16_t *__restrict__ lrow)
{
  const int64_t g = (int64_t)blockIdx.x * blockDim.x + threadIdx.x;
  if (g >= groups) return;
  const v4u d = *(const v4u *)(lrow8 + g * kBinGroup);
  unsigned r = gbase[g];
  unsigned out[kBinGroup / 2];
#pragma unroll
  for (int j = 0; j < kBinGroup; j += 2) {
    const unsigned w = j < 4 ? d.x : j < 8 ? d.y : j < 12 ? d.z : d.w;
    const unsigned a = r + ((w >> (8 * (j & 3))) & 0xffu), b = a + ((w >> (8 * ((j + 1) & 3))) & 0xffu);
    out[j / 2] = a | (b << 16);
    r = b;
  }
#pragma unroll
  for (int j = 0; j < kBinGroup / 8; ++j)
    *(v4u *)(lrow + g * kBinGroup + 8 * j) = v4u{out[4 * j], out[4 * j + 1], out[4 * j + 2], out[4 * j + 3]};
}

static void ensure_two_byte_ids(BinnedCsr &N, hipStream_t s)
{
  if (N.lrow || !N.lrow8 || N.lrow_tried) return;
  hipStreamCaptureStatus cap = hipStreamCaptureStatusNone;
  if (hipStreamIsCapturing(s, &cap) != hipSuccess) { (void)hipGetLastError(); return; }
  if (cap != hipStreamCaptureStatusNone) return;
  N.lrow_tried = true;
  uint16_t *p = nullptr;
  if (hipMalloc(&p, sizeof(uint16_t) * (size_t)N.n) != hipSuccess) { (void)hipGetLastError(); return; }
  const int64_t groups = N.n >> kBinGroupLog;
  if (groups > 0) hipLaunchKernelGGL(rows8_decode_kernel, dim3((unsigned)((groups + 255) / 256)), dim3(256), 0, s, groups, N.lrow8, N.gbase, p);
  if (hipGetLastError() != hipSuccess || hipStreamSynchronize(s) != hipSuccess) { (void)hipGetLastError(); (void)hipFree(p); return; }
  N.lrow = p;
}

static void launch_reduce(const BinnedCsr &N, double *out, int os, int p0, int p1, int flags, hipStream_t s)
{
#define FS_REDUCE(NT, RM, L8)                                                                                               \
  hipLaunchKernelGGL((spmv_reduce_kernel<NT, RM, L8>), dim3(p1 - p0), dim3(kBinBlock), 0, s, N.bin_ptr, N.panel_row, N.lrow, \
                     N.prod, out, os, p0, N.lrow8, N.gbase)
#define FS_REDUCE2(RM, L8) do { if (flags & 256) FS_REDUCE(false, RM, L8); else FS_REDUCE(true, RM, L8); } while (0)
  if (N.bcols == kBinColsBig) FS_REDUCE2(kBinRowsBig, false);
  else if (N.lrow8)           FS_REDUCE2(kBinRowsMax, true);
  else                        FS_REDUCE2(kBinRowsMax, false);
#undef FS_REDUCE2
#undef FS_REDUCE
}

int launch_spmv_binned(const DeviceCsr &A, double *y, const double *x, hipStream_t s, int xs, int ys, int p0, int p1, int row0,
                       int row1)
{
  const BinnedCsr &N = *A.binned;
  double *out = N.split ? N.yv : y;
  const int os = N.split ? 1 : ys;
  const bool part = p1 >= 0;
  if (!part) { p0 = 0; p1 = N.P; row0 = 0; row1 = A.nrow; }
  const int nwg1 = (options().bin_wgs > 0 && options().bin_wgs < N.nwg1) ? options().bin_wgs : N.nwg1;
  if (nwg1 > 0 && p0 == 0) {
    const int flags = options().bin_flags;
#define FS_EXPAND4(V, U)                                                                                          \
  do {                                                                                                            \
    if (flags & 16) { if (flags & 8) FS_EXPAND(V, U, true, false);  else FS_EXPAND(V, U, true, true); }           \
    else            { if (flags & 8) FS_EXPAND(V, U, false, false); else FS_EXPAND(V, U, false, true); }          \
  } while (0)
#define FS_EXPAND(V, U, NL, NS)                                                                                    \
  hipLaunchKernelGGL((spmv_expand_kernel<V, U, NL, NS>), dim3(nwg1), dim3(kBinBlock), 0, s, A.ncol, N.B, N.band_ptr, \
                     N.lcol, N.vals, N.gdst, x, xs, N.prod, 0u, (unsigned)(N.n >> kBinGroupLog))
    if (N.bcols == kBinColsBig) {
      if (A.has_vals())
        hipLaunchKernelGGL((spmv_expand_kernel<true, 4, false, true, kBinColsBig>), dim3(nwg1), dim3(kBinBlock), 0, s, A.ncol, N.B,
                           N.band_ptr, N.lcol, N.vals, N.gdst, x, xs, N.prod, 0u, (unsigned)(N.n >> kBinGroupLog));
      else
        hipLaunchKernelGGL((spmv_expand_kernel<false, 4, false, true, kBinColsBig>), dim3(nwg1), dim3(kBinBlock), 0, s, A.ncol, N.B,
                           N.band_ptr, N.lcol, N.vals, N.gdst, x, xs, N.prod, 0u, (unsigned)(N.n >> kBinGroupLog));
    } else
    if (A.has_vals()) { if ((flags & 3) == 1) FS_EXPAND4(true, 8); else if ((flags & 3) == 2) FS_EXPAND4(true, 2); else FS_EXPAND4(true, 4); }
    else        { if ((flags & 3) == 1) FS_EXPAND4(false, 8); else if ((flags & 3) == 2) FS_EXPAND4(false, 2); else FS_EXPAND4(false, 4); }
#undef FS_EXPAND4
#undef FS_EXPAND
    FS_HIP(hipGetLastError());
  }
  if (N.lr && p0 == 0)
    if (int rc = launch_longrows(A, *N.lr, x, xs, s)) return rc;
  if (p1 > p0) {
    const bool ordered = reproducible_now() || (options().bin_flags & 32);
    if (ordered && N.lrow8 && !N.lrow) ensure_two_byte_ids(*A.binned, s);
    if (N.bcols == kBinColsBig && ordered)
      hipLaunchKernelGGL((spmv_reduce_ordered_kernel<false, kBinRowsBig, FS_ORDERED_DEPTH>), dim3(p1 - p0), dim3(64), 0, s, N.bin_ptr,
                         N.panel_row, N.lrow, N.prod, out, os, p0);
    else if (ordered && N.lrow8 && !N.lrow)
      hipLaunchKernelGGL((spmv_reduce_ordered_kernel<false, kBinRowsMax, FS_ORDERED_DEPTH, true>), dim3(p1 - p0), dim3(64), 0, s, N.bin_ptr,
                         N.panel_row, N.lrow, N.prod, out, os, p0, N.lrow8, N.gbase);
    else if (ordered)
      hipLaunchKernelGGL((spmv_reduce_ordered_kernel<false, kBinRowsMax, FS_ORDERED_DEPTH>), dim3(p1 - p0), dim3(64), 0, s, N.bin_ptr,
                         N.panel_row, N.lrow, N.prod, out, os, p0);
    else
      launch_reduce(N, out, os, p0, p1, options().bin_flags, s);
    FS_HIP(hipGetLastError());
  }
  if (N.split && row1 > row0) {
    if (int rc = launch_tiled_combine(row1, N.vfirst, N.yv, y, ys, row0, s)) return rc;
  }
  if (N.lr && row1 > row0) {
    hipLaunchKernelGGL(longrows_scatter_kernel, dim3((unsigned)((N.lr->nlong + kBlock - 1) / kBlock)), dim3(kBlock), 0, s, N.lr->nlong,
                       N.lr->row, N.lr->ylong, y, ys, row0, row1);
    FS_HIP(hipGetLastError());
  }
  return FS_OK;
}

int launch_expand_groups(const DeviceCsr &A, const double *x, unsigned g0, unsigned g1, int wgs, hipStream_t s)
{
  const BinnedCsr &N = *A.binned;
  if (g1 <= g0 || wgs <= 0) return FS_OK;
#define FS_XH(V, BC)                                                                                                    \
  hipLaunchKernelGGL((spmv_expand_kernel<V, 4, false, true, BC>), dim3(wgs), dim3(kBinBlock), 0, s, A.ncol, N.B, N.band_ptr, \
                     N.lcol, N.vals, N.gdst, x, 1, N.prod, g0, g1)
  if (N.bcols == kBinColsBig) { if (A.has_vals()) FS_XH(true, kBinColsBig); else FS_XH(false, kBinColsBig); }
  else                        { if (A.has_vals()) FS_XH(true, kBinCols); else FS_XH(false, kBinCols); }
#undef FS_XH
  FS_HIP(hipGetLastError());
  return FS_OK;
}

int launch_reduce_panels(const DeviceCsr &A, double *y, int p0, int p1, hipStream_t s)
{
  const BinnedCsr &N = *A.binned;
  if (p1 <= p0) return FS_OK;
  launch_reduce(N, y, 1, p0, p1, 0, s);
  FS_HIP(hipGetLastError());
  return FS_OK;
}

int launch_spmm_binned(const DeviceCsr &A, const BinnedCsr &N, double *Y, const double *X, hipStream_t s, int xs, int ys, int p0,
                       int p1, int row0, int row1)
{
  const int K = N.kw;
  double *out = N.split ? N.yv : Y;
  const int os = N.split ? K : ys;
  if (p1 < 0) { p0 = 0; p1 = N.P; row0 = 0; row1 = A.nrow; }
  const int nwg1 = (p0 != 0) ? 0 : ((options().bin_wgs > 0 && options().bin_wgs < N.nwg1) ? options().bin_wgs : N.nwg1);
#define FS_XP(V, KK)                                                                                                  \
  hipLaunchKernelGGL((spmm_expand_kernel<V, KK, 4>), dim3(nwg1), dim3(kBinBlock), 0, s, A.ncol, N.B, N.band_ptr, N.lcol, \
                     N.vals, N.gdst, X, xs, N.prod)
  if (nwg1 > 0) {
    if (K == 2) { if (A.has_vals()) FS_XP(true, 2); else FS_XP(false, 2); }
    else        { if (A.has_vals()) FS_XP(true, 4); else FS_XP(false, 4); }
    FS_HIP(hipGetLastError());
  }
#undef FS_XP
  if (p1 > p0) {
    const bool ordered = reproducible_now() || (options().bin_flags & 32);
    if (K == 2 && ordered)
      hipLaunchKernelGGL((spmm_reduce_ordered_kernel<2, FS_ORDERED_DEPTH>), dim3(p1 - p0), dim3(64), 0, s, N.bin_ptr, N.panel_row, N.lrow, N.prod, out, os, p0);
    else if (ordered)
      hipLaunchKernelGGL((spmm_reduce_ordered_kernel<4, FS_ORDERED_DEPTH>), dim3(p1 - p0), dim3(64), 0, s, N.bin_ptr, N.panel_row, N.lrow, N.prod, out, os, p0);
    else if (K == 2)
      hipLaunchKernelGGL(spmm_reduce_kernel<2>, dim3(p1 - p0), dim3(kBinBlock), 0, s, N.bin_ptr, N.panel_row, N.lrow, N.prod, out, os, p0);
    else
      hipLaunchKernelGGL(spmm_reduce_kernel<4>, dim3(p1 - p0), dim3(kBinBlock), 0, s, N.bin_ptr, N.panel_row, N.lrow, N.prod, out, os, p0);
    FS_HIP(hipGetLastError());
  }
  if (N.split && row1 > row0) {
    const unsigned grid = (unsigned)(((int64_t)(row1 - row0) * K + kBlock - 1) / kBlock);
    if (K == 2)
      hipLaunchKernelGGL(tiled_combine_k_kernel<2>, dim3(grid), dim3(kBlock), 0, s, row1, N.vfirst, N.yv, Y, ys, row0);
    else
      hipLaunchKernelGGL(tiled_combine_k_kernel<4>, dim3(grid), dim3(kBlock), 0, s, row1, N.vfirst, N.yv, Y, ys, row0);
    FS_HIP(hipGetLastError());
  }
  return FS_OK;
}

}
```

Measured before the change: 2537.

## Store binned values in reduce order and multiply in reduce pass

The binned two-pass SpMV and SpMM now lay out matrix values in the panel (reduce) order instead of the band (expand) order. The value multiply moves from the expand kernel into the reduce kernels, so expand only gathers x into prod. This shrinks expand traffic and lets the values stream contiguously alongside prod in reduce. In exchange the reduce kernels carry more register pressure, which is why the ordered prefetch depth is lowered for valued matrices.

```diff
diff --git a/libfastsparse_amd/csrc/fs_copies.hip b/libfastsparse_amd/csrc/fs_copies.hip
--- a/libfastsparse_amd/csrc/fs_copies.hip
+++ b/libfastsparse_amd/csrc/fs_copies.hip
@@ -742,7 +742,7 @@
                                    const int *__restrict__ panel_row, const int *__restrict__ cols,
                                    const double *__restrict__ vals, const int *__restrict__ run_ptr,
                                    const unsigned *__restrict__ start1, const unsigned *__restrict__ start2,
-                                   uint16_t *__restrict__ lcol, double *__restrict__ vals1, uint16_t *__restrict__ lrow)
+                                   uint16_t *__restrict__ lcol, double *__restrict__ vals2, uint16_t *__restrict__ lrow)
 {
   const int64_t i = (int64_t)blockIdx.x * blockDim.x + threadIdx.x;
   if (i >= nnz) return;
@@ -752,7 +752,7 @@
   const int64_t pos1 = (int64_t)start1[key] * ge + rank;
   const int64_t pos2 = (int64_t)start2[(int64_t)p * B + b] * ge + rank;
   lcol[pos1] = (uint16_t)(cols[src] - b * bcols);
-  if (vals) vals1[pos1] = vals[src];
+  if (vals) vals2[pos2] = vals[src];
   lrow[pos2] = (uint16_t)(vrows[src] - panel_row[p]);
 }
 
@@ -776,7 +776,7 @@
                                     const int *__restrict__ panel_row, const int *__restrict__ cols,
                                     const double *__restrict__ vals, const int *__restrict__ run_ptr,
                                     const unsigned *__restrict__ xs, const unsigned *__restrict__ start1,
-                                    const unsigned *__restrict__ start2, uint16_t *__restrict__ lcol, double *__restrict__ vals1,
+                                    const unsigned *__restrict__ start2, uint16_t *__restrict__ lcol, double *__restrict__ vals2,
                                     uint8_t *__restrict__ lrow8, uint16_t *__restrict__ gbase)
 {
   const int64_t i = (int64_t)blockIdx.x * blockDim.x + threadIdx.x;
@@ -796,7 +796,7 @@
   }
   const int before = prev + 255 * (int)dum;
   lcol[base1 + slot] = (uint16_t)(cols[src] - b * bcols);
-  if (vals) vals1[base1 + slot] = vals[src];
+  if (vals) vals2[base2 + slot] = vals[src];
   lrow8[base2 + slot] = (uint8_t)(row - before);
   if ((slot & (ge - 1)) == 0) gbase[(base2 + slot) / ge] = (uint16_t)before;
 }
diff --git a/libfastsparse_amd/csrc/fs_kernels_twopass.hip b/libfastsparse_amd/csrc/fs_kernels_twopass.hip
--- a/libfastsparse_amd/csrc/fs_kernels_twopass.hip
+++ b/libfastsparse_amd/csrc/fs_kernels_twopass.hip
@@ -5,11 +5,11 @@
 namespace fs {
 
 
-template <bool VALUED, int U, bool NTLD, bool NTST, int BC>
+template <int U, bool NTLD, bool NTST, int BC>
 __device__ __forceinline__ void expand_share(double *__restrict__ xband, int ncol, int B, const unsigned *__restrict__ band_ptr,
-                                             const uint16_t *__restrict__ lcol, const double *__restrict__ vals,
-                                             const unsigned *__restrict__ gdst, const double *__restrict__ x, int xs,
-                                             double *__restrict__ prod, unsigned g0, unsigned g1)
+                                             const uint16_t *__restrict__ lcol, const unsigned *__restrict__ gdst,
+                                             const double *__restrict__ x, int xs, double *__restrict__ prod, unsigned g0,
+                                             unsigned g1)
 {
   const int t = threadIdx.x;
   if (g0 >= g1) return;
@@ -48,49 +48,43 @@
     int64_t o = e0 + 2 * t;
     for (; o - 2 * t + kRound <= e1; o += kRound) {
       unsigned a[U], d[U];
-      v2d v[U];
 #pragma unroll
       for (int k = 0; k < U; ++k) {
         const int64_t e = o + (int64_t)k * 2 * kBinBlock;
         a[k] = stream_load<NTLD>((const unsigned *)(lcol + e));
         d[k] = stream_load<NTLD>(gdst + (e >> kBinGroupLog));
-        if (VALUED) v[k] = stream_load<NTLD>((const v2d *)(vals + e));
       }
       __builtin_amdgcn_sched_barrier(0);
 #pragma unroll
       for (int k = 0; k < U; ++k) {
         const int64_t e = o + (int64_t)k * 2 * kBinBlock;
-        v2d p = {xband[a[k] & 0xffffu], xband[a[k] >> 16]};
-        if (VALUED) { p.x *= v[k].x; p.y *= v[k].y; }
+        const v2d p = {xband[a[k] & 0xffffu], xband[a[k] >> 16]};
         stream_store<NTST>(p, (v2d *)(prod + (int64_t)d[k] * kBinGroup + (e & (kBinGroup - 1))));
       }
     }
     for (; o < e1; o += 2 * kBinBlock) {
       const unsigned a = stream_load<NTLD>((const unsigned *)(lcol + o));
       const unsigned d = stream_load<NTLD>(gdst + (o >> kBinGroupLog));
-      v2d p = {xband[a & 0xffffu], xband[a >> 16]};
-      if (VALUED) {
-        const v2d v = stream_load<NTLD>((const v2d *)(vals + o));
-        p.x *= v.x; p.y *= v.y;
-      }
+      const v2d p = {xband[a & 0xffffu], xband[a >> 16]};
       stream_store<NTST>(p, (v2d *)(prod + (int64_t)d * kBinGroup + (o & (kBinGroup - 1))));
     }
     g = gb;
   }
 }
 
-template <bool VALUED, int U, bool NTLD, bool NTST, int BC = kBinCols>
+template <int U, bool NTLD, bool NTST, int BC = kBinCols>
 __global__ __launch_bounds__(kBinBlock) void spmv_expand_kernel(
     int ncol, int B, const unsigned *__restrict__ band_ptr, const uint16_t *__restrict__ lcol,
-    const double *__restrict__ vals, const unsigned *__restrict__ gdst, const double *__restrict__ x, int xs,
-    double *__restrict__ prod, unsigned gbeg, unsigned gend)
+    const unsigned *__restrict__ gdst, const double *__restrict__ x, int xs, double *__restrict__ prod, unsigned gbeg,
+    unsigned gend)
 {
   __shared__ double xband[BC + 8];
   const uint64_t groups = gend - gbeg;
   const unsigned g0 = gbeg + (unsigned)(groups * blockIdx.x / gridDim.x), g1 = gbeg + (unsigned)(groups * (blockIdx.x + 1) / gridDim.x);
-  expand_share<VALUED, U, NTLD, NTST, BC>(xband, ncol, B, band_ptr, lcol, vals, gdst, x, xs, prod, g0, g1);
-}
-
+  expand_share<U, NTLD, NTST, BC>(xband, ncol, B, band_ptr, lcol, gdst, x, xs, prod, g0, g1);
+}
+
+static_assert(kBinGroupLog == 4, "the one-byte row ids (row_ids, line_ids, rows8_decode_kernel) decode groups of 16 entries: two lanes of 8, eight lanes of 2, four words of 4");
 template <bool NTLD, bool L8>
 __device__ __forceinline__ v4u row_ids_load(const uint16_t *__restrict__ lrow, const uint8_t *__restrict__ lrow8,
                                             const uint16_t *__restrict__ gbase, int64_t e)
@@ -134,11 +128,12 @@
   return (off + d0) | ((off + own) << 16);
 }
 
-template <bool NTLD, bool L8 = false>
+template <bool VALUED, bool NTLD, bool L8 = false>
 __device__ __forceinline__ void reduce_panel(double *__restrict__ ytile, int panel, const unsigned *__restrict__ bin_ptr,
                                              const int *__restrict__ panel_row, const uint16_t *__restrict__ lrow,
-                                             const double *__restrict__ prod, double *__restrict__ y, int ys,
-                                             const uint8_t *__restrict__ lrow8 = nullptr, const uint16_t *__restrict__ gbase = nullptr)
+                                             const double *__restrict__ vals, const double *__restrict__ prod, double *__restrict__ y,
+                                             int ys, const uint8_t *__restrict__ lrow8 = nullptr,
+                                             const uint16_t *__restrict__ gbase = nullptr)
 {
   const int t = threadIdx.x;
   const int r0 = panel_row[panel], nr = panel_row[panel + 1] - r0;
@@ -153,7 +148,7 @@
   for (; eb + kRound <= e1; eb += kRound) {
     const int64_t e = eb + lane0;
     unsigned a[2][4];
-    v2d p[2][4];
+    v2d p[2][4], v[2][4];
 #pragma unroll
     for (int k = 0; k < 2; ++k)
 #pragma unroll
@@ -161,6 +156,7 @@
         const int64_t ek = e + k * kStep + 128 * j;
         a[k][j] = line_ids_load<L8>(lrow, lrow8, gbase, ek);
         p[k][j] = stream_load<NTLD>((const v2d *)(prod + ek));
+        if (VALUED) v[k][j] = stream_load<NTLD>((const v2d *)(vals + ek));
       }
     __builtin_amdgcn_sched_barrier(0);
 #pragma unroll
@@ -168,22 +164,25 @@
 #pragma unroll
       for (int j = 0; j < 4; ++j) {
         const unsigned r = line_ids<L8>(a[k][j]);
+        if (VALUED) { p[k][j].x *= v[k][j].x; p[k][j].y *= v[k][j].y; }
         FS_ADD2(r, p[k][j])
       }
   }
   for (; eb + wave0 < e1; eb += kStep) {
     const int64_t e = eb + lane0;
     unsigned a[4];
-    v2d p[4];
+    v2d p[4], v[4];
 #pragma unroll
     for (int j = 0; j < 4; ++j) {
       const int64_t ej = e + 128 * j, ec = ej < e1 ? ej : e1 - 2;
       a[j] = line_ids_load<L8>(lrow, lrow8, gbase, ec);
       p[j] = stream_load<NTLD>((const v2d *)(prod + ec));
+      if (VALUED) v[j] = stream_load<NTLD>((const v2d *)(vals + ec));
     }
 #pragma unroll
     for (int j = 0; j < 4; ++j) {
       const unsigned r = line_ids<L8>(a[j]);
+      if (VALUED) { p[j].x *= v[j].x; p[j].y *= v[j].y; }
       if (e + 128 * j < e1) { FS_ADD2(r, p[j]) }
     }
   }
@@ -193,24 +192,27 @@
   for (int i = t; i < nr; i += kBinBlock) y[(int64_t)(r0 + i) * ys] = ytile[i];
 }
 
-template <bool NTLD, int RM = kBinRowsMax, bool L8 = false>
+template <bool VALUED, bool NTLD, int RM = kBinRowsMax, bool L8 = false>
 __global__ __launch_bounds__(kBinBlock) void spmv_reduce_kernel(
     const unsigned *__restrict__ bin_ptr, const int *__restrict__ panel_row, const uint16_t *__restrict__ lrow,
-    const double *__restrict__ prod, double *__restrict__ y, int ys, int pbase, const uint8_t *__restrict__ lrow8 = nullptr,
-    const uint16_t *__restrict__ gbase = nullptr)
+    const double *__restrict__ vals, const double *__restrict__ prod, double *__restrict__ y, int ys, int pbase,
+    const uint8_t *__restrict__ lrow8 = nullptr, const uint16_t *__restrict__ gbase = nullptr)
 {
   __shared__ double ytile[RM];
-  reduce_panel<NTLD, L8>(ytile, pbase + blockIdx.x, bin_ptr, panel_row, lrow, prod, y, ys, lrow8, gbase);
+  reduce_panel<VALUED, NTLD, L8>(ytile, pbase + blockIdx.x, bin_ptr, panel_row, lrow, vals, prod, y, ys, lrow8, gbase);
 }
 
 #ifndef FS_ORDERED_DEPTH
 #define FS_ORDERED_DEPTH 16
 #endif
-template <bool NTLD, int RM, int DEPTH, bool L8 = false>
+#ifndef FS_ORDERED_DEPTH_VALUED
+#define FS_ORDERED_DEPTH_VALUED 10
+#endif
+template <bool VALUED, bool NTLD, int RM, int DEPTH, bool L8 = false>
 __global__ __launch_bounds__(64) void spmv_reduce_ordered_kernel(
     const unsigned *__restrict__ bin_ptr, const int *__restrict__ panel_row, const uint16_t *__restrict__ lrow,
-    const double *__restrict__ prod, double *__restrict__ y, int ys, int pbase, const uint8_t *__restrict__ lrow8 = nullptr,
-    const uint16_t *__restrict__ gbase = nullptr)
+    const double *__restrict__ vals, const double *__restrict__ prod, double *__restrict__ y, int ys, int pbase,
+    const uint8_t *__restrict__ lrow8 = nullptr, const uint16_t *__restrict__ gbase = nullptr)
 {
   __shared__ __attribute__((aligned(16))) double ytile[RM];
   const int t = threadIdx.x;
@@ -226,12 +228,15 @@
   FS_ADD(A.w & 0xffffu, P[3].x); FS_ADD(A.w >> 16, P[3].y);
   constexpr int64_t kStep = 8 * 64;
   v4u a[DEPTH];
-  v2d p[DEPTH][4];
+  v2d p[DEPTH][4], v[VALUED ? DEPTH : 1][4];
   auto fetch = [&](int k, int64_t e) {
     const int64_t ec = (e + 8 <= e1) ? e : (e1 - e0 >= 8 ? e1 - 8 : e0);
     a[k] = row_ids_load<NTLD, L8>(lrow, lrow8, gbase, ec);
 #pragma unroll
-    for (int j = 0; j < 4; ++j) p[k][j] = stream_load<NTLD>((const v2d *)(prod + ec + 2 * j));
+    for (int j = 0; j < 4; ++j) {
+      p[k][j] = stream_load<NTLD>((const v2d *)(prod + ec + 2 * j));
+      if (VALUED) v[k][j] = stream_load<NTLD>((const v2d *)(vals + ec + 2 * j));
+    }
   };
   if (e1 > e0) {
     int64_t e = e0 + 8 * t;
@@ -243,6 +248,10 @@
         const int64_t ek = e + (int64_t)k * kStep;
         const v4u ak = row_ids<L8>(a[k]);
         v2d pk[4] = {p[k][0], p[k][1], p[k][2], p[k][3]};
+        if (VALUED) {
+#pragma unroll
+          for (int j = 0; j < 4; ++j) { pk[j].x *= v[k][j].x; pk[j].y *= v[k][j].y; }
+        }
         fetch(k, ek + (int64_t)DEPTH * kStep);
         if (ek + 8 <= e1) { FS_ADD8(ak, pk) }
       }
@@ -398,11 +407,10 @@
 }
 
 
-template <bool VALUED, int K, int U>
+template <int K, int U>
 __global__ __launch_bounds__(kBinBlock) void spmm_expand_kernel(
     int ncol, int B, const unsigned *__restrict__ band_ptr, const uint16_t *__restrict__ lcol,
-    const double *__restrict__ vals, const unsigned *__restrict__ gdst, const double *__restrict__ X, int xs,
-    double *__restrict__ prod)
+    const unsigned *__restrict__ gdst, const double *__restrict__ X, int xs, double *__restrict__ prod)
 {
   constexpr int BC = kBinCols / K;
   constexpr int GE = kBinGroup / K;
@@ -449,38 +457,34 @@
     int64_t o = e0 + le;
     for (; o - le + kRound <= e1; o += kRound) {
       unsigned a[U], d[U];
-      double v[U];
 #pragma unroll
       for (int k = 0; k < U; ++k) {
         const int64_t e = o + (int64_t)k * EPS;
         a[k] = lcol[e];
         d[k] = gdst[e / GE];
-        if (VALUED) v[k] = vals[e];
       }
       __builtin_amdgcn_sched_barrier(0);
 #pragma unroll
       for (int k = 0; k < U; ++k) {
         const int64_t e = o + (int64_t)k * EPS;
-        v2d p = *reinterpret_cast<const v2d *>(&xband[a[k] * K + 2 * h]);
-        if (VALUED) { p.x *= v[k]; p.y *= v[k]; }
+        const v2d p = *reinterpret_cast<const v2d *>(&xband[a[k] * K + 2 * h]);
         __builtin_nontemporal_store(p, (v2d *)(prod + ((int64_t)d[k] * GE + (e % GE)) * K + 2 * h));
       }
     }
     for (; o < e1; o += EPS) {
       const unsigned a = lcol[o];
       const unsigned d = gdst[o / GE];
-      v2d p = *reinterpret_cast<const v2d *>(&xband[a * K + 2 * h]);
-      if (VALUED) { const double v = vals[o]; p.x *= v; p.y *= v; }
+      const v2d p = *reinterpret_cast<const v2d *>(&xband[a * K + 2 * h]);
       __builtin_nontemporal_store(p, (v2d *)(prod + ((int64_t)d * GE + (o % GE)) * K + 2 * h));
     }
     g = gb;
   }
 }
 
-template <int K>
+template <bool VALUED, int K>
 __global__ __launch_bounds__(kBinBlock) void spmm_reduce_kernel(
     const unsigned *__restrict__ bin_ptr_all, const int *__restrict__ panel_row_all, const uint16_t *__restrict__ lrow,
-    const double *__restrict__ prod, double *__restrict__ Y, int ys, int pbase)
+    const double *__restrict__ vals, const double *__restrict__ prod, double *__restrict__ Y, int ys, int pbase)
 {
   const unsigned *__restrict__ bin_ptr = bin_ptr_all + pbase;
   const int *__restrict__ panel_row = panel_row_all + pbase;
@@ -493,15 +497,18 @@
   __syncthreads();
   const int64_t e0 = (int64_t)bin_ptr[blockIdx.x] * GE, e1 = (int64_t)bin_ptr[blockIdx.x + 1] * GE;
   typedef uint16_t rows_t __attribute__((ext_vector_type(EPL)));
+  typedef double vals_t __attribute__((ext_vector_type(EPL)));
 #define FS_ADD(idx, val) __hip_atomic_fetch_add(&ytile[idx], val, __ATOMIC_RELAXED, __HIP_MEMORY_SCOPE_WORKGROUP)
-  auto add8 = [&](const rows_t a, const v2d (&p)[4]) {
+  auto add8 = [&](const rows_t a, const v2d (&p)[4], const vals_t v) {
 #pragma unroll
     for (int q = 0; q < EPL; ++q) {
       const int base = (int)a[q] * K;
 #pragma unroll
       for (int j = 0; j < K; j += 2) {
-        FS_ADD(base + j, p[(q * K + j) / 2].x);
-        FS_ADD(base + j + 1, p[(q * K + j) / 2].y);
+        v2d t2 = p[(q * K + j) / 2];
+        if (VALUED) { t2.x *= v[q]; t2.y *= v[q]; }
+        FS_ADD(base + j, t2.x);
+        FS_ADD(base + j + 1, t2.y);
       }
     }
   };
@@ -511,33 +518,37 @@
   for (; e - EPL * t + kRound <= e1; e += kRound) {
     rows_t a[2];
     v2d p[2][4];
+    vals_t v[2] = {};
 #pragma unroll
     for (int k = 0; k < 2; ++k) {
       const int64_t ek = e + k * kStep;
       a[k] = *reinterpret_cast<const rows_t *>(lrow + ek);
+      if (VALUED) v[k] = *reinterpret_cast<const vals_t *>(vals + ek);
 #pragma unroll
       for (int j = 0; j < 4; ++j) p[k][j] = *reinterpret_cast<const v2d *>(prod + ek * K + 2 * j);
     }
     __builtin_amdgcn_sched_barrier(0);
-    add8(a[0], p[0]);
-    add8(a[1], p[1]);
+    add8(a[0], p[0], v[0]);
+    add8(a[1], p[1], v[1]);
   }
   for (; e < e1; e += kStep) {
     const rows_t a = *reinterpret_cast<const rows_t *>(lrow + e);
+    vals_t v = {};
+    if (VALUED) v = *reinterpret_cast<const vals_t *>(vals + e);
     v2d p[4];
 #pragma unroll
     for (int j = 0; j < 4; ++j) p[j] = *reinterpret_cast<const v2d *>(prod + e * K + 2 * j);
-    add8(a, p);
+    add8(a, p, v);
   }
 #undef FS_ADD
   __syncthreads();
   for (int i = t; i < nr * K; i += kBinBlock) Y[(int64_t)(r0 + i / K) * ys + (i % K)] = ytile[i];
 }
 
-template <int K, int DEPTH>
+template <bool VALUED, int K, int DEPTH>
 __global__ __launch_bounds__(64) void spmm_reduce_ordered_kernel(
     const unsigned *__restrict__ bin_ptr_all, const int *__restrict__ panel_row_all, const uint16_t *__restrict__ lrow,
-    const double *__restrict__ prod, double *__restrict__ Y, int ys, int pbase)
+    const double *__restrict__ vals, const double *__restrict__ prod, double *__restrict__ Y, int ys, int pbase)
 {
   const unsigned *__restrict__ bin_ptr = bin_ptr_all + pbase;
   const int *__restrict__ panel_row = panel_row_all + pbase;
@@ -549,24 +560,29 @@
   for (int i = t; i < nr * K; i += 64) ytile[i] = 0.0;
   const int64_t e0 = (int64_t)bin_ptr[blockIdx.x] * GE, e1 = (int64_t)bin_ptr[blockIdx.x + 1] * GE;
   typedef uint16_t rows_t __attribute__((ext_vector_type(EPL)));
+  typedef double vals_t __attribute__((ext_vector_type(EPL)));
 #define FS_ADD(idx, val) __hip_atomic_fetch_add(&ytile[idx], val, __ATOMIC_RELAXED, __HIP_MEMORY_SCOPE_WORKGROUP)
-  auto add8 = [&](const rows_t a, const v2d (&p)[4]) {
+  auto add8 = [&](const rows_t a, const v2d (&p)[4], const vals_t v) {
 #pragma unroll
     for (int q = 0; q < EPL; ++q) {
       const int base = (int)a[q] * K;
 #pragma unroll
       for (int j = 0; j < K; j += 2) {
-        FS_ADD(base + j, p[(q * K + j) / 2].x);
-        FS_ADD(base + j + 1, p[(q * K + j) / 2].y);
+        v2d t2 = p[(q * K + j) / 2];
+        if (VALUED) { t2.x *= v[q]; t2.y *= v[q]; }
+        FS_ADD(base + j, t2.x);
+        FS_ADD(base + j + 1, t2.y);
       }
     }
   };
   constexpr int64_t kStep = (int64_t)EPL * 64;
   rows_t a[DEPTH];
   v2d p[DEPTH][4];
+  vals_t v[VALUED ? DEPTH : 1] = {};
   auto fetch = [&](int k, int64_t e) {
     const int64_t ec = (e + EPL <= e1) ? e : (e1 - e0 >= EPL ? e1 - EPL : e0);
     a[k] = *reinterpret_cast<const rows_t *>(lrow + ec);
+    if (VALUED) v[k] = *reinterpret_cast<const vals_t *>(vals + ec);
 #pragma unroll
     for (int j = 0; j < 4; ++j) p[k][j] = *reinterpret_cast<const v2d *>(prod + ec * K + 2 * j);
   };
@@ -580,8 +596,9 @@
         const int64_t ek = e + (int64_t)k * kStep;
         const rows_t ak = a[k];
         const v2d pk[4] = {p[k][0], p[k][1], p[k][2], p[k][3]};
+        const vals_t vk = v[VALUED ? k : 0];
         fetch(k, ek + (int64_t)DEPTH * kStep);
-        if (ek + EPL <= e1) add8(ak, pk);
+        if (ek + EPL <= e1) add8(ak, pk, vk);
       }
     }
   }
@@ -642,10 +659,14 @@
 
 static void launch_reduce(const BinnedCsr &N, double *out, int os, int p0, int p1, int flags, hipStream_t s)
 {
-#define FS_REDUCE(NT, RM, L8)                                                                                               \
-  hipLaunchKernelGGL((spmv_reduce_kernel<NT, RM, L8>), dim3(p1 - p0), dim3(kBinBlock), 0, s, N.bin_ptr, N.panel_row, N.lrow, \
-                     N.prod, out, os, p0, N.lrow8, N.gbase)
-#define FS_REDUCE2(RM, L8) do { if (flags & 256) FS_REDUCE(false, RM, L8); else FS_REDUCE(true, RM, L8); } while (0)
+#define FS_REDUCE(V, NT, RM, L8)                                                                                                \
+  hipLaunchKernelGGL((spmv_reduce_kernel<V, NT, RM, L8>), dim3(p1 - p0), dim3(kBinBlock), 0, s, N.bin_ptr, N.panel_row, N.lrow, \
+                     N.vals, N.prod, out, os, p0, N.lrow8, N.gbase)
+#define FS_REDUCE2(RM, L8)                                                                       \
+  do {                                                                                           \
+    if (N.vals) { if (flags & 256) FS_REDUCE(true, false, RM, L8); else FS_REDUCE(true, true, RM, L8); }   \
+    else        { if (flags & 256) FS_REDUCE(false, false, RM, L8); else FS_REDUCE(false, true, RM, L8); } \
+  } while (0)
   if (N.bcols == kBinColsBig) FS_REDUCE2(kBinRowsBig, false);
   else if (N.lrow8)           FS_REDUCE2(kBinRowsMax, true);
   else                        FS_REDUCE2(kBinRowsMax, false);
@@ -664,24 +685,20 @@
   const int nwg1 = (options().bin_wgs > 0 && options().bin_wgs < N.nwg1) ? options().bin_wgs : N.nwg1;
   if (nwg1 > 0 && p0 == 0) {
     const int flags = options().bin_flags;
-#define FS_EXPAND4(V, U)                                                                                          \
-  do {                                                                                                            \
-    if (flags & 16) { if (flags & 8) FS_EXPAND(V, U, true, false);  else FS_EXPAND(V, U, true, true); }           \
-    else            { if (flags & 8) FS_EXPAND(V, U, false, false); else FS_EXPAND(V, U, false, true); }          \
+#define FS_EXPAND4(U)                                                                                       \
+  do {                                                                                                      \
+    if (flags & 16) { if (flags & 8) FS_EXPAND(U, true, false);  else FS_EXPAND(U, true, true); }           \
+    else            { if (flags & 8) FS_EXPAND(U, false, false); else FS_EXPAND(U, false, true); }          \
   } while (0)
-#define FS_EXPAND(V, U, NL, NS)                                                                                    \
-  hipLaunchKernelGGL((spmv_expand_kernel<V, U, NL, NS>), dim3(nwg1), dim3(kBinBlock), 0, s, A.ncol, N.B, N.band_ptr, \
-                     N.lcol, N.vals, N.gdst, x, xs, N.prod, 0u, (unsigned)(N.n >> kBinGroupLog))
-    if (N.bcols == kBinColsBig) {
-      if (A.has_vals())
-        hipLaunchKernelGGL((spmv_expand_kernel<true, 4, false, true, kBinColsBig>), dim3(nwg1), dim3(kBinBlock), 0, s, A.ncol, N.B,
-                           N.band_ptr, N.lcol, N.vals, N.gdst, x, xs, N.prod, 0u, (unsigned)(N.n >> kBinGroupLog));
-      else
-        hipLaunchKernelGGL((spmv_expand_kernel<false, 4, false, true, kBinColsBig>), dim3(nwg1), dim3(kBinBlock), 0, s, A.ncol, N.B,
-                           N.band_ptr, N.lcol, N.vals, N.gdst, x, xs, N.prod, 0u, (unsigned)(N.n >> kBinGroupLog));
-    } else
-    if (A.has_vals()) { if ((flags & 3) == 1) FS_EXPAND4(true, 8); else if ((flags & 3) == 2) FS_EXPAND4(true, 2); else FS_EXPAND4(true, 4); }
-    else        { if ((flags & 3) == 1) FS_EXPAND4(false, 8); else if ((flags & 3) == 2) FS_EXPAND4(false, 2); else FS_EXPAND4(false, 4); }
+#define FS_EXPAND(U, NL, NS)                                                                                      \
+  hipLaunchKernelGGL((spmv_expand_kernel<U, NL, NS>), dim3(nwg1), dim3(kBinBlock), 0, s, A.ncol, N.B, N.band_ptr, \
+                     N.lcol, N.gdst, x, xs, N.prod, 0u, (unsigned)(N.n >> kBinGroupLog))
+    if (N.bcols == kBinColsBig)
+      hipLaunchKernelGGL((spmv_expand_kernel<4, false, true, kBinColsBig>), dim3(nwg1), dim3(kBinBlock), 0, s, A.ncol, N.B,
+                         N.band_ptr, N.lcol, N.gdst, x, xs, N.prod, 0u, (unsigned)(N.n >> kBinGroupLog));
+    else if ((flags & 3) == 1) FS_EXPAND4(8);
+    else if ((flags & 3) == 2) FS_EXPAND4(2);
+    else                       FS_EXPAND4(4);
 #undef FS_EXPAND4
 #undef FS_EXPAND
     FS_HIP(hipGetLastError());
@@ -691,17 +708,21 @@
   if (p1 > p0) {
     const bool ordered = reproducible_now() || (options().bin_flags & 32);
     if (ordered && N.lrow8 && !N.lrow) ensure_two_byte_ids(*A.binned, s);
-    if (N.bcols == kBinColsBig && ordered)
-      hipLaunchKernelGGL((spmv_reduce_ordered_kernel<false, kBinRowsBig, FS_ORDERED_DEPTH>), dim3(p1 - p0), dim3(64), 0, s, N.bin_ptr,
-                         N.panel_row, N.lrow, N.prod, out, os, p0);
-    else if (ordered && N.lrow8 && !N.lrow)
-      hipLaunchKernelGGL((spmv_reduce_ordered_kernel<false, kBinRowsMax, FS_ORDERED_DEPTH, true>), dim3(p1 - p0), dim3(64), 0, s, N.bin_ptr,
-                         N.panel_row, N.lrow, N.prod, out, os, p0, N.lrow8, N.gbase);
-    else if (ordered)
-      hipLaunchKernelGGL((spmv_reduce_ordered_kernel<false, kBinRowsMax, FS_ORDERED_DEPTH>), dim3(p1 - p0), dim3(64), 0, s, N.bin_ptr,
-                         N.panel_row, N.lrow, N.prod, out, os, p0);
+#define FS_ORDERED(RM, L8)                                                                                                     \
+  do {                                                                                                                         \
+    if (N.vals)                                                                                                                \
+      hipLaunchKernelGGL((spmv_reduce_ordered_kernel<true, false, RM, FS_ORDERED_DEPTH_VALUED, L8>), dim3(p1 - p0), dim3(64), 0, s, \
+                         N.bin_ptr, N.panel_row, N.lrow, N.vals, N.prod, out, os, p0, N.lrow8, N.gbase);                       \
+    else                                                                                                                       \
+      hipLaunchKernelGGL((spmv_reduce_ordered_kernel<false, false, RM, FS_ORDERED_DEPTH, L8>), dim3(p1 - p0), dim3(64), 0, s,  \
+                         N.bin_ptr, N.panel_row, N.lrow, N.vals, N.prod, out, os, p0, N.lrow8, N.gbase);                       \
+  } while (0)
+    if (N.bcols == kBinColsBig && ordered)  FS_ORDERED(kBinRowsBig, false);
+    else if (ordered && N.lrow8 && !N.lrow) FS_ORDERED(kBinRowsMax, true);
+    else if (ordered)                       FS_ORDERED(kBinRowsMax, false);
     else
       launch_reduce(N, out, os, p0, p1, options().bin_flags, s);
+#undef FS_ORDERED
     FS_HIP(hipGetLastError());
   }
   if (N.split && row1 > row0) {
@@ -719,11 +740,11 @@
 {
   const BinnedCsr &N = *A.binned;
   if (g1 <= g0 || wgs <= 0) return FS_OK;
-#define FS_XH(V, BC)                                                                                                    \
-  hipLaunchKernelGGL((spmv_expand_kernel<V, 4, false, true, BC>), dim3(wgs), dim3(kBinBlock), 0, s, A.ncol, N.B, N.band_ptr, \
-                     N.lcol, N.vals, N.gdst, x, 1, N.prod, g0, g1)
-  if (N.bcols == kBinColsBig) { if (A.has_vals()) FS_XH(true, kBinColsBig); else FS_XH(false, kBinColsBig); }
-  else                        { if (A.has_vals()) FS_XH(true, kBinCols); else FS_XH(false, kBinCols); }
+#define FS_XH(BC)                                                                                                         \
+  hipLaunchKernelGGL((spmv_expand_kernel<4, false, true, BC>), dim3(wgs), dim3(kBinBlock), 0, s, A.ncol, N.B, N.band_ptr, \
+                     N.lcol, N.gdst, x, 1, N.prod, g0, g1)
+  if (N.bcols == kBinColsBig) FS_XH(kBinColsBig);
+  else                        FS_XH(kBinCols);
 #undef FS_XH
   FS_HIP(hipGetLastError());
   return FS_OK;
@@ -746,25 +767,28 @@
   const int os = N.split ? K : ys;
   if (p1 < 0) { p0 = 0; p1 = N.P; row0 = 0; row1 = A.nrow; }
   const int nwg1 = (p0 != 0) ? 0 : ((options().bin_wgs > 0 && options().bin_wgs < N.nwg1) ? options().bin_wgs : N.nwg1);
-#define FS_XP(V, KK)                                                                                                  \
-  hipLaunchKernelGGL((spmm_expand_kernel<V, KK, 4>), dim3(nwg1), dim3(kBinBlock), 0, s, A.ncol, N.B, N.band_ptr, N.lcol, \
-                     N.vals, N.gdst, X, xs, N.prod)
+#define FS_XP(KK)                                                                                                  \
+  hipLaunchKernelGGL((spmm_expand_kernel<KK, 4>), dim3(nwg1), dim3(kBinBlock), 0, s, A.ncol, N.B, N.band_ptr, N.lcol, \
+                     N.gdst, X, xs, N.prod)
   if (nwg1 > 0) {
-    if (K == 2) { if (A.has_vals()) FS_XP(true, 2); else FS_XP(false, 2); }
-    else        { if (A.has_vals()) FS_XP(true, 4); else FS_XP(false, 4); }
+    if (K == 2) FS_XP(2); else FS_XP(4);
     FS_HIP(hipGetLastError());
   }
 #undef FS_XP
   if (p1 > p0) {
     const bool ordered = reproducible_now() || (options().bin_flags & 32);
-    if (K == 2 && ordered)
-      hipLaunchKernelGGL((spmm_reduce_ordered_kernel<2, FS_ORDERED_DEPTH>), dim3(p1 - p0), dim3(64), 0, s, N.bin_ptr, N.panel_row, N.lrow, N.prod, out, os, p0);
-    else if (ordered)
-      hipLaunchKernelGGL((spmm_reduce_ordered_kernel<4, FS_ORDERED_DEPTH>), dim3(p1 - p0), dim3(64), 0, s, N.bin_ptr, N.panel_row, N.lrow, N.prod, out, os, p0);
-    else if (K == 2)
-      hipLaunchKernelGGL(spmm_reduce_kernel<2>, dim3(p1 - p0), dim3(kBinBlock), 0, s, N.bin_ptr, N.panel_row, N.lrow, N.prod, out, os, p0);
-    else
-      hipLaunchKernelGGL(spmm_reduce_kernel<4>, dim3(p1 - p0), dim3(kBinBlock), 0, s, N.bin_ptr, N.panel_row, N.lrow, N.prod, out, os, p0);
+#define FS_RP(V, KK)                                                                                                            \
+  do {                                                                                                                          \
+    if (ordered)                                                                                                                \
+      hipLaunchKernelGGL((spmm_reduce_ordered_kernel<V, KK, (V && KK == 2) ? 12 : FS_ORDERED_DEPTH>), dim3(p1 - p0), dim3(64), 0, s, N.bin_ptr, \
+                         N.panel_row, N.lrow, N.vals, N.prod, out, os, p0);                                                     \
+    else                                                                                                                        \
+      hipLaunchKernelGGL((spmm_reduce_kernel<V, KK>), dim3(p1 - p0), dim3(kBinBlock), 0, s, N.bin_ptr, N.panel_row, N.lrow,     \
+                         N.vals, N.prod, out, os, p0);                                                                          \
+  } while (0)
+    if (K == 2) { if (N.vals) FS_RP(true, 2); else FS_RP(false, 2); }
+    else        { if (N.vals) FS_RP(true, 4); else FS_RP(false, 4); }
+#undef FS_RP
     FS_HIP(hipGetLastError());
   }
   if (N.split && row1 > row0) {
```

New measurement: 2689 (median of 6 runs). 1.06x the previous value.
